# david3684/Prompt-Diffusion

Hardware: AMD Instinct MI355X
Metric: images/sec @ 512x512, 50-step DDIM, bs=8 (higher is better)
Workload: dtype f16; 1 GPU; SD1.5 UNet + Prompt-Diffusion ControlNet, 512x512, 50-step DDIM (eta 0), CFG 7.5, bs=8 per GPU (forward batch 16), random-init weights; global_batch=8, ddim_steps=50, parallelism=batch-shard x1, stream_f32=False, controlnet_stream_overlap=True

## Files before the change

### include/pdengine_ops.h

```cpp
#ifndef PDENGINE_OPS_H
#define PDENGINE_OPS_H
#include "pdengine.h"
#ifdef __cplusplus
extern "C" {
#endif
int pd_op_conv2d(pd_engine* e, const float* x, const float* w, const float* bias, const float* residual, int B, int Cin, int H,
                 int W, int Cout, int k, int stride, int upsample, int act_silu, float scale, int stream_out, float* y);
int pd_op_conv2d_upfold(pd_engine* e, const float* x, const float* w, const float* bias, const float* residual, int B, int Cin, int H,
                        int W, int Cout, float* y);
int pd_op_linear(pd_engine* e, const float* x, const float* w, const float* bias, int M, int K, int N, int geglu, int a_silu,
                 float* y);
typedef struct pd_gemm_ex_args {
    const float *x, *w, *bias, *residual, *rowvec, *gate, *ln_gamma, *ln_beta;
    int32_t M, K, N, act, a_silu, res_dt, out_dt, rows_per_sample;
    int32_t vt_begin, vt_extra, vt_tok_off, c_sample_rows, c_row_off, a_sample_rows, a_row_off, ldc_extra;
    float scale;
    float *y, *vt;
    int64_t touched;
} pd_gemm_ex_args;
int pd_op_linear_ex(pd_engine* e, pd_gemm_ex_args* a);
int pd_op_conv2d_ex(pd_engine* e, const float* x, const float* w, const float* bias, const float* residual, const float* rowvec, int B, int Cin,
                    int H, int W, int Cout, int k, int stride, int upsample, int act, float scale, int stream_out, float* y);
int pd_op_linear_fp8(pd_engine* e, const float* x, const float* w, const float* bias, int M, int K, int N, int act, float* y);
int pd_op_groupnorm(pd_engine* e, const float* x, const float* gamma, const float* beta, int B, int C, int H, int W, float eps,
                    int silu, float* y);
int pd_op_layernorm(pd_engine* e, const float* x, const float* gamma, const float* beta, int rows, int C, float* y);
int pd_op_groupnorm_slabs(pd_engine* e, const float* slabs, int nslab, const float* bias, const float* row, const float* gamma,
                          const float* beta, int B, int C, int H, int W, float eps, int silu, float* y);
int pd_op_groupnorm_coef(pd_engine* e, const float* x, const float* gamma, const float* beta, int B, int C, int H, int W, float eps,
                         float* coef);
int pd_op_ln_linear(pd_engine* e, int mode, const float* h, const float* x, const float* w1, const float* b1, const float* residual,
                    const float* gamma, const float* beta, const float* w, const float* bias, int M, int K, int N, float* h_out, float* y,
                    int* stats_parts, float* row_stats);
int pd_op_attention(pd_engine* e, const float* q, const float* k, const float* v, int B, int Nq, int Nk, int C, float* o);
int pd_op_attention_ex(pd_engine* e, const float* q, const float* k, const float* v, int B, int Nq, int Nk, int C, int heads, int causal,
                       float scale, const float* relbias, int layout, int vt_extra, float pad_fill, float* o, int64_t* touched);
int pd_op_vae_attention(pd_engine* e, const float* q, const float* k, const float* v, int B, int N, int C, float* o);
int pd_op_spatial_transformer(pd_engine* e, const char* prefix, const float* x, const float* context, int B, int H, int W, float* y);
int pd_op_spatial_transformer_ctx(pd_engine* e, const char* prefix, const float* x, const float* context, int B, int H, int W, int L, float* y);
int pd_op_time_embed(pd_engine* e, int net, const int64_t* t, int n, float* temb, float* emb);
int pd_op_timestep_embedding_i(const int64_t* t, int n, int dim, float* out);
int pd_op_timestep_embedding_f(const double* t, int n, int dim, float* out);
int pd_op_vae_downsample(pd_engine* e, const float* x, const float* w, const float* bias, int B, int C, int H, int W, float* y);
int pd_op_freeu_concat(pd_engine* e, const float* h, const float* h_add, const float* skip, const float* skip_add, int B, int C_h,
                       int C_skip, int H, int W, int skip_B, int skip_add_B, float s, float b, float* y);
int pd_op_hed_stage_tail(pd_engine* e, const float* x, const float* w, const float* bias, int B, int C, int H, int W, float* score,
                         float* pooled);
int pd_op_hed_fuse(pd_engine* e, const float* scores, const float* cw, const float* cb, int B, int H, int W, int what, float* out);
int pd_op_canny_hysteresis(pd_engine* e, const uint8_t* states, int B, int H, int W, int mem, uint8_t* out);
int pd_op_dwconv3x3(pd_engine* e, const float* x, const float* w, const float* bias, int B, int C, int H, int W, int stride, int in_relu6,
                    float* y);
int pd_op_upcat_bilinear(pd_engine* e, const float* x, int B, int C, int h, int w, int Cy, int c_off, float* y);
int pd_op_conv2d_dilated(pd_engine* e, const float* x, const float* w, const float* bias, int B, int Cin, int H, int W, int Cout, int dilation,
                         int relu, float* y);
int pd_op_mlsd_decode(pd_engine* e, const float* tp, int B, int h, int w, float thr_v, float thr_d, int32_t* segs, int32_t* count);
int pd_op_draw_lines(pd_engine* e, const int32_t* segs, const int32_t* count, int B, int n, int H, int W, uint8_t* out);
int pd_op_vae_tile_blend(pd_engine* e, const float* tiles, const pd_vae_tile* plan, int rows, int cols, int B, int C, int Cpad, int nchw,
                         float* out);
int pd_op_sd3_update(pd_engine* e, const float* v, const float* x, const float* z0, const float* mask, const float* eps, int B, int C,
                     int H, int W, int use_cfg, float guidance, float dsigma, float sigma, int pure, int seeded, int mem, float* x_out,
                     float* x_in_out);
#ifdef __cplusplus
}
#endif
#endif
```

### prompt-diffusion_amd/csrc/engine.cpp

```cpp
#include "engine.h"

#include <algorithm>
#include <climits>
#include <cmath>
#include <cstdarg>
#include <cstdio>
#include <cstring>

static thread_local char g_err[1024] = "";
void pd_set_error(const char* fmt, ...) {
    va_list ap;
    va_start(ap, fmt);
    vsnprintf(g_err, sizeof(g_err), fmt, ap);
    va_end(ap);
}
const char* pd_err_buf() { return g_err; }

static inline int round_up(int x, int m) { return (x + m - 1) / m * m; }

void* pd_engine::dmalloc(size_t bytes) {
    void* p = nullptr;
    if (bytes == 0) bytes = 16;
    if (hipMalloc(&p, bytes) != hipSuccess) { alloc_failed = true; return nullptr; }
    hipMemset(p, 0, bytes);
// ... 858 lines not shown

int pd_engine::gemm(const WMat& m, const Act& in, Act& out, const GemmCall& c) {
    PD_TRY(check_gemm(m, in, out, c));
    GemmParams p = fill_gemm(m, in, out, c);
    GemmPlan pl = plan_gemm(p, m, c);
    if (c.defer) c.defer->active = false;
    if (c.gn_coef && !pl.patch()) { pd_set_error("internal: fused GroupNorm requested for a conv that is not patch-eligible"); return 1; }
    const size_t mk = arena.mark();
    if (pl.splitk > 1) {
        p.slab = arena.alloc((size_t)pl.splitk * p.M * m.N * sizeof(float));
        if (!arena.dry && arena.top > arena.cap) {
            if (pl.patch()) { pd_set_error("no workspace for the conv split-K slabs"); return 1; }
            p.slab = nullptr; arena.overflow = false;
            pl = plan_gemm(p, m, c, false);
        }
    }
    p.splitk = pl.splitk; p.big_tile = pl.big_tile; p.defer_finalize = pl.defer_finalize ? 1 : 0;
    p.tile_cnt = pl.fused_tile_cnt ? tile_cnt : nullptr;
    if (pl.defer_finalize) c.defer->active = true;
    else arena.release(mk);
    if (pl.stats_parts) {
        LnStats& st = *c.ln_out;
        st.parts = p.stats_parts = pl.stats_parts; st.C = m.Nout; p.stats_out = st.stats;
        if (st.cap_parts && st.parts > st.cap_parts) { pd_set_error("internal: %d LayerNorm statistics partials per row, buffer holds %d", st.parts, st.cap_parts); return 1; }
    }
    if (arena.dry) return 0;
    PD_TRY(check_arena());
    const bool gemv = pl.family == GEMM_GEMV, ring = pl.family == GEMM_RING;
    ++launches;
    gemm_family = pl.family; gemm_splitk = p.splitk;
    gemm_ring_tile = ring ? pl.ring_tile : -1;
    gemm_tile = pl.family == GEMM_IGEMM ? gemm_launched_tile(p, in.dt == DT_FP8 ? PREC_FP8 : P) : 0;
    if (opt.gemm_tile >= 0 && pl.family == GEMM_IGEMM && gemm_tile != opt.gemm_tile) {
        pd_set_error("gemm: option gemm_tile %d, but this launch (mode, operands, epilogue, %d slices) has the tile %d instantiation only", opt.gemm_tile, p.splitk, gemm_tile);
        return 1;
    }
    ProfRec rec{};
    if (profiling && gemv) {
        prof_begin(rec, 1, 2.0 * (double)p.M * (double)m.Nout * (double)m.cin);
        rec.M = p.M; rec.N = p.N; rec.K = p.K; rec.taps = 10;
    } else if (profiling) {
        const double n_log = m.geglu ? 2.0 * m.Nout : (double)m.Nout;
        const bool upfold = pl.family == GEMM_UPFOLD;
        prof_begin(rec, pl.patch() || upfold ? 3 : m.taps == 9 ? 0 : 1, 2.0 * (double)p.M * n_log * (double)(upfold ? 4 : m.taps) * (double)m.cin);
        rec.M = p.M; rec.N = p.N; rec.K = upfold ? 4 * p.Cin : p.K; rec.taps = (upfold ? 4 : p.taps) * 10 + p.stride + (p.ups ? 5 : 0);
    }
    hipEvent_t mid = (profiling && !gemv && !pl.patch() && pl.family != GEMM_UPFOLD) ? next_event() : nullptr;
    if (gemv) {
        const int r = launch_gemv(reinterpret_cast<const float*>(in.p), in.C, m.w, T, m.Kpad, m.bias, reinterpret_cast<float*>(out.p), p.ldc,
                                  p.M, m.N, m.K, p.a_silu, stream);
        if (profiling) prof_end(rec);
        if (r) { pd_set_error("gemv launch failed"); return 1; }
        return 0;
    }
    static const char* const family_name[] = {"gemv", "patch1", "patch2", "patch4", "ring", "igemm", "upfold"};
    if (opt.verbose >= 2)
        fprintf(stderr, "[pdengine] gemm M %d N %d K %d taps %d stride %d ups %d: %s splitk %d big_tile %d ring_tile %d act %d R %d ln_in %d ln_out %d\n", p.M, p.N, p.K, p.taps,
                p.stride, p.ups, family_name[pl.family], p.splitk, p.big_tile, pl.ring_tile, p.act, p.R ? 1 : 0, p.ln_stats ? 1 : 0, p.stats_out ? 1 : 0);
    const int prec = in.dt == DT_FP8 ? PREC_FP8 : P;
    const int r = pl.family == GEMM_UPFOLD ? launch_conv_upfold(p, m.w_up, P, stream) : pl.family == GEMM_PATCH4 ? launch_conv_patch4(p, P, stream) : pl.family == GEMM_PATCH2 ? launch_conv_patch2(p, P, stream) :
                  pl.family == GEMM_PATCH1 ? launch_conv_patch(p, P, stream) : ring ? launch_ring_gemm(p, prec, pl.ring_tile, ncu, stream) : launch_gemm(p, prec, stream, mid);
    if (r) { pd_set_error("gemm launch failed: %s", hipGetErrorString(hipGetLastError())); return 1; }
    if (ring) ++ring_launches;
    if (pl.family == GEMM_UPFOLD) ++ups_fold_launches;
    if (pl.defer_finalize) *c.defer = SlabDefer{true, true, reinterpret_cast<const float*>(p.slab), p.splitk, p.bias, p.rowvec, p.rowvec_stride};
    if (profiling && mid && ring) HIP_OK(hipEventRecord(mid, stream));
    if (profiling) {
        if (mid) { rec.b = mid; prof.push_back(rec); }
        else prof_end(rec);
    }
    if (c.ln_out && !p.stats_out) {
        c.ln_out->parts = 1; c.ln_out->C = m.Nout;
        ++launches;
        if (launch_row_stats(out.p, out.dt, c.ln_out->stats, (int)out.rows(), out.C, stream)) { pd_set_error("row statistics launch failed"); return 1; }
    }
    return 0;
}

int pd_engine::conv(const ConvW& c, const Act& in, Act& out, GemmCall call) {
    call.stride = c.stride; call.pad_shift = c.pad_shift; call.dilation = c.dilation;
    return gemm(c.m, in, out, call);
}

int pd_engine::gn_stats(const Act& x, int& nchunk) {
    const int HW = x.H * x.W;
    nchunk = HW / 8;
    if (nchunk < 1) nchunk = 1;
    if (nchunk > 64) nchunk = 64;
    while ((size_t)x.B * nchunk * 32 * 2 * sizeof(double) > gn_partial_cap && nchunk > 1) nchunk /= 2;
    PD_LAUNCH(this, launch_gn_stats(x.p, x.dt, gn_partial, x.B, HW, x.C, 32, nchunk, stream), "groupnorm stats launch failed (C=%d)", x.C);
    return 0;
}

int pd_engine::groupnorm(const Act& x, Act& y, const float* g, const float* b, float eps, bool silu, const SlabDefer* from_slabs) {
    if (from_slabs && from_slabs->active) {
        if (!(opt.gn_single && gn_fused_bundle(x.dt, x.H * x.W, x.C, 32, opt.gn_reg))) { pd_set_error("internal: deferred split-K slabs without the single-kernel GroupNorm"); return 1; }
        if (arena.dry) return 0;
        PD_TRY(check_arena());
        ++launches;
        ++gn_from_slabs;
        if (launch_gn_fused_slabs(from_slabs->slabs, from_slabs->nslab, from_slabs->bias, from_slabs->rowvec, from_slabs->rowvec_stride, x.dt, y.p, y.dt, g, b,
                                  x.B, x.H * x.W, x.C, 32, eps, silu ? 1 : 0, opt.gn_reg, stream, &gn_kernel)) {
            pd_set_error("groupnorm (single kernel, split-K slabs) launch failed (C=%d)", x.C);
            return 1;
        }
        return 0;
    }
    if (opt.gn_single && gn_fused_bundle(x.dt, x.H * x.W, x.C, 32, opt.gn_reg)) {
        PD_LAUNCH(this, launch_gn_fused(x.p, x.dt, y.p, y.dt, g, b, x.B, x.H * x.W, x.C, 32, eps, silu ? 1 : 0, opt.gn_reg, stream, &gn_kernel),
                  "groupnorm (single kernel) launch failed (C=%d)", x.C);
        return 0;
    }
    int nchunk = 1;
    PD_TRY(gn_stats(x, nchunk));
    if (arena.dry) return 0;
    ++launches;
    gn_kernel = GN_KIND_TWO_PASS;
    if (launch_gn_apply(x.p, x.dt, y.p, y.dt, gn_partial, g, b, x.B, x.H * x.W, x.C, 32, nchunk, eps, silu ? 1 : 0, stream)) {
        pd_set_error("groupnorm launch failed (C=%d)", x.C);
        return 1;
    }
    return 0;
}

int pd_engine::conv_gn(const ConvW& c, const Act& x, Act& out, const float* g, const float* b, float eps, bool silu, GemmCall call,
                       const SlabDefer* in_slabs) {
    call.stride = c.stride; call.pad_shift = c.pad_shift; call.dilation = c.dilation;
    const bool fuse = opt.gn_fuse && x.C == c.m.cin_pad && patch_unsplit(patch_tiles(fill_gemm(c.m, x, out, call)));
    if (!fuse) {
        const size_t mk = arena.mark();
        Act a = new_act(x.B, x.H, x.W, x.C, T);
        PD_TRY(groupnorm(x, a, g, b, eps, silu, in_slabs));
        PD_TRY(gemm(c.m, a, out, call));
        if (!(call.defer && call.defer->active)) arena.release(mk);
        return 0;
    }
    if (in_slabs && in_slabs->active) { pd_set_error("internal: deferred split-K slabs in front of a GroupNorm-fused conv"); return 1; }
    int nchunk = 1;
    PD_TRY(gn_stats(x, nchunk));
    const size_t mk = arena.mark();
    float* coef = reinterpret_cast<float*>(arena.alloc((size_t)x.B * x.C * 2 * sizeof(float)));
    PD_LAUNCH(this, launch_gn_coef(gn_partial, g, b, coef, x.B, x.H * x.W, x.C, 32, nchunk, eps, stream), "groupnorm coefficient launch failed");
    call.gn_coef = coef; call.gn_silu = silu; call.defer = nullptr;
    PD_TRY(gemm(c.m, x, out, call));
    arena.release(mk);
    return 0;
}

int pd_engine::layernorm(const Act& x, Act& y, const float* g, const float* b, float eps) {
    PD_LAUNCH(this, launch_layernorm(x.p, x.dt, y.p, y.dt, g, b, (int)x.rows(), x.C, eps, stream), "layernorm launch failed (C=%d)", x.C);
    return 0;
}

int pd_engine::attention(const void* Q, int ldq, const void* K, int ldk, const void* VT, int vt_ld, void* O, int ldo, int B,
                         int Nq, int Nk, int C, int heads, bool causal, long long q_bs, long long k_bs, long long o_bs, const float* relbias,
                         float scale) {
    if (heads <= 0) heads = cfg.num_heads;
    if (arena.dry) return 0;
    PD_TRY(check_arena());
    AttnParams p{};
    p.Q = Q; p.K = K; p.VT = VT; p.O = O;
    p.ldq = ldq; p.ldk = ldk; p.ldo = ldo; p.vt_ld = vt_ld;
    p.q_bs = q_bs ? q_bs : (long long)Nq * ldq;
    p.k_bs = k_bs ? k_bs : (long long)Nk * ldk;
    p.vt_bs = (long long)C * vt_ld;
    p.o_bs = o_bs ? o_bs : (long long)Nq * ldo;
    p.Nq = Nq; p.Nk = Nk; p.heads = heads; p.dh = C / heads;
    p.causal = causal ? 1 : 0;
    p.scale = (float)(1.0 / std::sqrt((double)p.dh));
    if (scale != 0.f) p.scale = scale;
    p.B = B;
    p.legacy = opt.attn_legacy ? 1 : 0;
    ++launches;
    ProfRec rec{};
    if (profiling) {
        prof_begin(rec, 2, 4.0 * (double)B * heads * (double)Nq * (double)Nk * (double)p.dh);
        rec.M = Nq; rec.N = Nk; rec.K = p.dh; rec.taps = B;
    }
    const int r = relbias ? launch_attention_bias(p, relbias, P, stream, &attn_kernel) : launch_attention(p, P, stream, &attn_kernel);
    if (profiling) prof_end(rec);
    if (r) {
        pd_set_error(r == 2 ? "attention: unsupported head dim %d" : "attention launch failed (dh %d)", p.dh);
        return 1;
    }
    return 0;
}

int pd_engine::resblock(const ResW& r, const Act& x, Act& out, const float* embrow, int emb_stride) {
    out = new_act(x.B, x.H, x.W, r.cout, S);
    const size_t mk = arena.mark();
    Act h = new_act(x.B, x.H, x.W, r.cout, T);
    SlabDefer d;
    d.allow = opt.slab_gn && !opt.gn_fuse && opt.gn_single && h.dt == T && gn_fused_bundle(T, x.H * x.W, r.cout, 32, opt.gn_reg) > 0;
    PD_TRY(conv_gn(r.conv1, x, h, r.gn1_g, r.gn1_b, r.eps, true, {.rowvec = embrow, .rowvec_stride = emb_stride, .defer = &d}));
    Act skip = x;
    if (r.has_skip) {
        skip = new_act(x.B, x.H, x.W, r.cout, S);
        PD_TRY(conv(r.skip, x, skip));
    }
    PD_TRY(conv_gn(r.conv2, h, out, r.gn2_g, r.gn2_b, r.eps, true, {.R = &skip}, &d));
    arena.release(mk);
    return 0;
}

int pd_engine::transformer(const STW& s, const Act& x, Act& out, const KVSlot& kv, int out_B) {
    int B = x.B;
    const int H = x.H, W = x.W, C = s.C, N = H * W;
    if (out_B <= 0) out_B = B;
    if (out_B % B) { pd_set_error("internal: transformer output batch %d over %d shared samples", out_B, B); return 1; }
    const int reps = out_B / B;
    out = new_act(out_B, H, W, C, S);
    const size_t mk = arena.mark();
    const int L = kv.L > 0 ? kv.L : cfg.context_len, lpad = round_up(L, 8);
    const bool fused = st_tail_on(s, N, L) && s.tail_w && s.front_w && kv.P;
    const int npad = round_up(N, 8);
    Act h, qk, vt, ln;
    LnStats st0, st1;
    const bool fuse = (opt.ln_fuse < 0 ? !f32 : opt.ln_fuse != 0) && s.qkv.w_ln != nullptr;
    if (fused) {
        int nchunk = 1;
        PD_TRY(gn_stats(x, nchunk));
        float* coef = reinterpret_cast<float*>(arena.alloc((size_t)B * C * 2 * sizeof(float)));
        h = new_act(B, H, W, C, S);
        qk = new_act(B, H, W, 2 * C, T);
        vt = new_act(B, C, 1, npad, T);
        if (!arena.dry) {
            PD_TRY(check_arena());
            launches += 2;
            if (launch_gn_coef(gn_partial, s.gn_g, s.gn_b, coef, B, N, C, 32, nchunk, 1e-6f, stream)) {
                pd_set_error("groupnorm coefficient launch failed");
                return 1;
            }
            ProfRec rec{};
            if (profiling) {
                prof_begin(rec, 4, st_front_flops((long long)B * N));
                rec.M = B * N; rec.N = 4 * C; rec.K = C; rec.taps = 1;
            }
            const int r = launch_st_front(x.p, coef, h.p, qk.p, vt.p, s.front_w, s.front_vec, (long long)B * N, N, npad, P, stream);
            if (profiling) prof_end(rec);
            if (r) { pd_set_error("fused transformer-front launch failed: %s", hipGetErrorString(hipGetLastError())); return 1; }
        }
    } else {
    Act a = new_act(B, H, W, C, T);
    PD_TRY(groupnorm(x, a, s.gn_g, s.gn_b, 1e-6f, false));
    if (fuse) {
        st0.cap_parts = st1.cap_parts = ((C + 159) / 160) * 2;
        const size_t cap = (size_t)B * N * (size_t)st0.cap_parts * 2 * sizeof(float);
        st0.stats = reinterpret_cast<float*>(arena.alloc(cap));
        st1.stats = reinterpret_cast<float*>(arena.alloc(cap));
    }
    h = new_act(B, H, W, C, S);
    PD_TRY(gemm(s.proj_in.m, a, h, {.ln_out = fuse ? &st0 : nullptr}));
    if (!fuse) {
        ln = new_act(B, H, W, C, T);
        PD_TRY(layernorm(h, ln, s.ln_g[0], s.ln_b[0]));
    }
    qk = new_act(B, H, W, 2 * C, T);
    vt = new_act(B, C, 1, npad, T);
    PD_TRY(gemm(s.qkv, fuse ? h : ln, qk, {.VT = vt.p, .vt_begin = 2 * C, .vt_ld = npad, .ln_in = fuse ? &st0 : nullptr}));
    }
    Act att = new_act(B, H, W, C, T);
    const size_t eb = dt_size(T);
    PD_TRY(attention(qk.p, 2 * C, reinterpret_cast<char*>(qk.p) + (size_t)C * eb, 2 * C, vt.p, npad, att.p, C, B, N, N, C));
    if (fused) {
        if (!arena.dry) {
            PD_TRY(check_arena());
            ++launches;
            ProfRec rec{};
            if (profiling) {
                prof_begin(rec, 4, st_tail_flops((long long)out_B * N, L));
                rec.M = out_B * N; rec.N = C; rec.K = C; rec.taps = 0;
            }
            const int r = launch_st_tail(att.p, h.p, x.p, out.p, s.tail_w, s.tail_vec, kv.P, (long long)out_B * N, N, L, S,
                                         (float)(1.0 / std::sqrt((double)(C / cfg.num_heads))), P, stream, (long long)B * N);
            if (profiling) prof_end(rec);
            if (r) { pd_set_error("fused transformer-tail launch failed: %s", hipGetErrorString(hipGetLastError())); return 1; }
        }
// ... 71 lines not shown
    auto ctl = [&](int i) { return s0 ? batch_view(ses.control[i], s0, Bf) : ses.control[i]; };
    for (size_t i = 0; i < n.enc.size(); ++i) {
        EncBlock& b = n.enc[i];
        Act o;
        if (b.kind == 0) {
            o = new_act(x_in.B, x_in.H, x_in.W, b.cout, S);
            PD_TRY(conv(b.conv, x_in, o, {.R = &hint}));
        } else if (b.kind == 2) {
            o = new_act(h.B, h.H / 2, h.W / 2, b.cout, S);
            PD_TRY(conv(b.conv, h, o));
        } else {
            PD_TRY(resblock(b.res, h, o, emb_ptr(ses.emb_c, b.res, emb_row), emb_stride ? b.res.cout : 0));
            if (b.attn) {
                Act o2;
                PD_TRY(transformer(b.st, o, o2, kvs(b.st), Bf));
                o = o2;
            }
        }
        h = o;
        Act c = ctl((int)i);
        if (c.B != h.B) { pd_set_error("internal: control tensor %d sized for batch %d, block output has %d", (int)i, c.B, h.B); return 1; }
        PD_TRY(conv(n.zero[i], h, c, {.scale = scales ? scales[i] : 1.f}));
    }
    Act m0, m1, m2;
    PD_TRY(resblock(n.mid0, h, m0, emb_ptr(ses.emb_c, n.mid0, emb_row), emb_stride ? n.mid0.cout : 0));
    PD_TRY(transformer(n.mid1, m0, m1, kvs(n.mid1), Bf));
    PD_TRY(resblock(n.mid2, m1, m2, emb_ptr(ses.emb_c, n.mid2, emb_row), emb_stride ? n.mid2.cout : 0));
    const int last = (int)n.enc.size();
    Act cl = ctl(last);
    PD_TRY(conv(n.mid_out, m2, cl, {.scale = scales ? scales[last] : 1.f}));
    return 0;
}

Act pd_engine::batch_view(const Act& a, int first, int count) {
    Act v = a;
    v.p = reinterpret_cast<char*>(a.p) + (size_t)first * a.H * a.W * a.C * dt_size(a.dt);
    v.B = count;
    return v;
}

int pd_engine::run_unet(const Act& x_in_full, int emb_row, int emb_stride, bool only_mid, Act& eps) {
    NetW& n = unet;
    std::vector<Act> hs;
    Act h;
    const int Bf = x_in_full.B;
    Act x_in = x_in_full;
    if (ses.share_u) x_in.B = Bf / 2;
    for (size_t i = 0; i < n.enc.size(); ++i) {
        EncBlock& b = n.enc[i];
        Act o;
        if (b.kind == 0) {
            o = new_act(x_in.B, x_in.H, x_in.W, b.cout, S);
            PD_TRY(conv(b.conv, x_in, o));
        } else if (b.kind == 2) {
            o = new_act(h.B, h.H / 2, h.W / 2, b.cout, S);
            PD_TRY(conv(b.conv, h, o));
        } else {
            PD_TRY(resblock(b.res, h, o, emb_ptr(ses.emb_u, b.res, emb_row), emb_stride ? b.res.cout : 0));
            if (b.attn) {
                Act o2;
                PD_TRY(transformer(b.st, o, o2, ses.kv_u[b.st.kv_slot], Bf));
                o = o2;
            }
        }
        h = o;
        hs.push_back(h);
    }
    Act m0, m1, m2;
    PD_TRY(resblock(n.mid0, h, m0, emb_ptr(ses.emb_u, n.mid0, emb_row), emb_stride ? n.mid0.cout : 0));
    PD_TRY(transformer(n.mid1, m0, m1, ses.kv_u[n.mid1.kv_slot], Bf));
    PD_TRY(resblock(n.mid2, m1, m2, emb_ptr(ses.emb_u, n.mid2, emb_row), emb_stride ? n.mid2.cout : 0));
    h = m2;
    PD_TRY(join_controlnet());
    const int nctl = (int)cnet.enc.size();
    for (size_t i = 0; i < n.dec.size(); ++i) {
        DecBlock& b = n.dec[i];
        Act skip = hs.back();
        hs.pop_back();
        Act cat = new_act(h.B, h.H, h.W, h.C + skip.C, S);
        const Act* a_add = i == 0 ? &ses.control[nctl] : nullptr;
        const Act* b_add = only_mid ? nullptr : &ses.control[nctl - 1 - (int)i];
        const int stage = (int)i / (cfg.num_res_blocks + 1);
        const bool fu = stage < 2 && freeu_on();
        PD_LAUNCH(this,
                  fu ? launch_freeu_concat(h.p, a_add ? a_add->p : nullptr, skip.p, b_add ? b_add->p : nullptr, cat.p, S, h.B, h.H, h.W, h.C, skip.C,
                                           freeu[stage], freeu[2 + stage], stream, skip.rows(), b_add ? b_add->rows() : 0)
                     : launch_concat_add(h.p, a_add ? a_add->p : nullptr, skip.p, b_add ? b_add->p : nullptr, cat.p, S, h.rows(), h.C, skip.C, stream,
                                         skip.rows(), b_add ? b_add->rows() : 0),
                  fu ? "FreeU concat launch failed" : "concat launch failed");
        Act o;
        PD_TRY(resblock(b.res, cat, o, emb_ptr(ses.emb_u, b.res, emb_row), emb_stride ? b.res.cout : 0));
        if (b.attn) {
            Act o2;
            PD_TRY(transformer(b.st, o, o2, ses.kv_u[b.st.kv_slot]));
            o = o2;
        }
        if (b.up) {
            Act o3 = new_act(o.B, o.H * 2, o.W * 2, o.C, S);
            PD_TRY(conv(b.upconv, o, o3, {.ups = 1}));
            o = o3;
        }
        h = o;
    }
    eps = new_act(h.B, h.H, h.W, round_up(cfg.out_channels, 4), DT_F32);
    PD_TRY(conv_gn(n.outconv, h, eps, n.out_g, n.out_b, 1e-5f, true));
    return 0;
}

void pd_engine::swap_context() {
    std::swap(arena, arena2);
    std::swap(stream, stream2);
    std::swap(gn_partial, gn_partial2);
    std::swap(tile_cnt, tile_cnt2);
}

int pd_engine::join_controlnet() {
    const pd_sample_args& a = ses.a;
    if (arena.dry) return 0;
    if (cn_pending) {
        HIP_OK(hipStreamWaitEvent(stream, ev_join, 0));
        cn_pending = false;
    }
    if (a.guess_mode && a.use_cfg) {
        for (size_t i = 0; i <= cnet.enc.size(); ++i)
            HIP_OK(hipMemsetAsync(ses.control[i].p, 0, ses.control[i].bytes() / 2, stream));
    }
    return 0;
}

int pd_engine::forward_eps(int emb_row, int emb_stride, const float* scales, Act& eps) {
    const pd_sample_args& a = ses.a;
    const int Bf = ses.Bf;
    Act x_in;
    x_in.p = ses.x_in; x_in.B = Bf; x_in.H = a.h; x_in.W = a.w; x_in.C = 8; x_in.dt = DT_F32;
    const bool share = opt.cfg_share && a.use_cfg && emb_stride == 0 && Bf % 2 == 0;
    ses.share_u = share;
    ses.share_c = share && ses.hint_shared && !a.guess_mode;
    ses.cn_cond_only = opt.cfg_share && a.guess_mode && a.use_cfg && emb_stride == 0 && Bf % 2 == 0;
    int hh = a.h, ww = a.w;
    bool front = ses.share_c;
    for (size_t i = 0; i < cnet.enc.size(); ++i) {
        if (cnet.enc[i].kind == 2) { hh /= 2; ww /= 2; }
        if (cnet.enc[i].attn) front = false;
        ses.control[i] = new_act(front ? Bf / 2 : Bf, hh, ww, cnet.enc[i].cout, S);
    }
    ses.control[cnet.enc.size()] = new_act(Bf, hh, ww, cnet.enc.back().cout, S);
    const bool two = opt.two_streams && stream2 != nullptr;
    if (two && !arena.dry) {
        HIP_OK(hipEventRecord(ev_fork, stream));
        HIP_OK(hipStreamWaitEvent(stream2, ev_fork, 0));
    }
    if (two) swap_context();
    const size_t mk = arena.mark();
    int rc = run_controlnet(x_in, emb_row, emb_stride, scales);
    arena.release(mk);
    if (two) {
        if (!rc && !arena.dry && hipEventRecord(ev_join, stream) != hipSuccess) rc = 1;
        swap_context();
    }
    if (rc) return rc;
    cn_pending = two;
    PD_TRY(run_unet(x_in, emb_row, emb_stride, a.only_mid_control != 0, eps));
    return 0;
}
```

### prompt-diffusion_amd/csrc/engine.h

```cpp
#pragma once
#include <cstdint>
#include <map>
#include <string>
#include <unordered_map>
#include <vector>

#include "../../include/pdengine.h"
#include "options.h"
#include "pd_common.h"

void pd_set_error(const char* fmt, ...);
void pd_host_timestep_embedding(const int64_t* t, int n, int dim, std::vector<float>& out);
void pd_host_timestep_embedding_f(const double* t, int n, int dim, std::vector<float>& out);
int pd_lms_table(const pd_config& cfg, const pd_lms_args& u, const int64_t* ts, int n, std::vector<double>& rows, std::vector<double>& times);
int pd_resample_axis(int in_size, int out_size, int filter, int* ksize, std::vector<int32_t>& bounds, std::vector<int32_t>& kk);
int pd_unipc_table(const pd_config& cfg, const pd_unipc_args& u, const int64_t* ts, int n, std::vector<double>& coef);

#define HIP_OK(expr)                                                                            \
    do {                                                                                        \
        hipError_t _e = (expr);                                                                 \
        if (_e != hipSuccess) {                                                                 \
            pd_set_error("%s failed: %s (%s:%d)", #expr, hipGetErrorString(_e), __FILE__, __LINE__); \
            return 1;                                                                           \
        }                                                                                       \
// ... 381 lines not shown
    float* x_state = nullptr;
    float* x_in = nullptr;
    float* pred_x0 = nullptr;
    float* eps_g = nullptr;
    float* noise = nullptr;
    bool noise_seeded = false;
    void* ctx = nullptr;
    Act hint;
    std::vector<KVSlot> kv_u, kv_c;
    std::vector<float*> emb_u, emb_c;
    int emb_rows = 0;
    float* per_step = nullptr;
    Act control[PD_NUM_CONTROL];
    size_t session_top = 0;
    bool hint_shared = false, share_u = false, share_c = false;
    bool cn_cond_only = false;
    int solver = 0;
    std::vector<double> unipc_coef;
    int unipc_ring = 0;
    double* u_last = nullptr;
    double* u_ring[3] = {nullptr, nullptr, nullptr};
    std::vector<double> lms_coef;
    std::vector<double> lms_times;
    std::vector<int> lms_step;
    std::vector<int> lms_pushed;
    int lms_ring = 0;
    bool lms_keep = false;
    double* l_keep = nullptr;
    double* l_ring[3] = {nullptr, nullptr, nullptr};
    int rows() const { return solver == SOLVER_LMS ? (int)lms_times.size() : S; }
    float* init_z0 = nullptr;
    float* init_eps = nullptr;
    float* mask = nullptr;
    std::vector<BlendCoef> blend;
};

struct pd_engine {
    pd_config cfg{};
    int device = 0;
    int ncu = 256;
    hipStream_t stream = nullptr;
    void* comm = nullptr;
    int comm_world = 1, comm_rank = 0;
    bool f32 = false;
    int P = DT_BF16;
    int T = DT_BF16;
    int S = DT_BF16;
    std::vector<Param> params;
    std::unordered_map<std::string, int> index;
    NetW unet, cnet;
    VaeW vae;
    VaeEncW vae_enc;
    ClipW text;
    struct GraphEntry { uint64_t key; hipGraph_t graph; hipGraphExec_t exec; };
    std::vector<GraphEntry> graphs;
    void clear_graphs();
    int run_steps_graph();
    WeightGroup reg_group = GROUP_SAMPLER;
    int missing(WeightGroup g) const;
    int require_loaded(WeightGroup g, const char* what);
    std::vector<void*> owned;
    bool alloc_failed = false;
    int check_arena();
    size_t weight_bytes = 0;
    Arena arena;
    Arena arena2;
    hipStream_t stream2 = nullptr;
    double* gn_partial2 = nullptr;
    int* tile_cnt2 = nullptr;
    hipEvent_t ev_fork = nullptr, ev_join = nullptr;
    bool cn_pending = false;
    EngineOptions opt;
    float freeu[4] = {0.f, 0.f, 0.f, 0.f};
    bool freeu_on() const { return freeu[0] != 0.f && freeu[1] != 0.f && freeu[2] != 0.f && freeu[3] != 0.f; }
    uint32_t* rng_dev = nullptr;
    uint32_t rng_host[4] = {0u, 0u, 0u, 0u};
    uint64_t rng_seed = 0, rng_base = 0;
    long long graph_captures = 0, graph_replays = 0;
    void swap_context();
    int join_controlnet();
    Session ses;
    long long launches = 0;
    long long gn_from_slabs = 0;
    long long ring_launches = 0;
    int gn_kernel = 0;
    long long ups_fold_launches = 0;
    int attn_kernel = 0;
    int gemm_tile = -1, gemm_splitk = -1;
    int gemm_ring_tile = -1;
    int gemm_family = -1;
    struct ProfRec { hipEvent_t a, b; int klass; double flops; int M, N, K, taps; };
    bool profiling = false;
    float prof_overhead_ms = 0.f;
    std::vector<ProfRec> prof;
    std::vector<hipEvent_t> ev_pool;
    size_t ev_used = 0;
    hipEvent_t next_event();
    void prof_begin(ProfRec& r, int klass, double flops);
    void prof_end(ProfRec& r);
    double* gn_partial = nullptr;
    int* tile_cnt = nullptr;
    static constexpr int kTileCnt = 4096;
    size_t gn_partial_cap = 0;

    int build();
    void* dmalloc(size_t bytes);
    void make_mat(WMat& m, int n_rows, int k_logical, int taps, int cin, bool bias, bool geglu = false);
    void reg_mat(const std::string& name, std::vector<int64_t> shape, WMat* m, int row_off, bool conv);
    void reg_vec(const std::string& name, int n, float** dst, char init);
    void reg_bias(const std::string& name, WMat* m, int off, int n, bool geglu = false);
    void build_conv(const std::string& prefix, ConvW& c, int cin, int cout, int k, int stride);
    void build_res(const std::string& prefix, ResW& r, int cin, int cout, NetW& net);
    void build_st(const std::string& prefix, STW& s, int ch, NetW& net);
    void build_encoder(const std::string& prefix, NetW& net);
    void build_middle(const std::string& prefix, NetW& net);
    void build_vres(const std::string& prefix, ResW& r, int cin, int cout, bool diffusers = false);
    void build_vattn(const std::string& prefix, VaeAttnW& a, int C, bool diffusers = false);
    void build_vae();
    void build_vae_encoder();
    void build_vae_decoder(VaeW& v, const std::string& prefix);
    void build_vae_encoder(VaeEncW& v, const std::string& prefix);
    VaeW sd3_vae;
    VaeEncW sd3_vae_enc;
    long long vae_flash_launches = 0;
    bool vae_flash_on(const VaeDesc& d, int C, long long N) const;
    int vae_forward(VaeW& v, const float* latents_dev, int B, int h, int w, float* out_dev, float scale, float shift);
    int vae_encoder_forward(VaeEncW& v, const float* images_dev, int B, int H, int W, int what, const float* noise_dev, float* out_dev, float scale,
                            float shift);
    int vae_attention(const VaeAttnW& a, const VaeDesc& d, const Act& x, Act& out);
    int vae_attn_product(const void* qk, int ld, const void* vt, int npad, void* att, int B, int N, int C, bool flash, float* sc, void* pr);
    int vae_decode_layers(VaeW& v, const Act& z, Act& img);
    int vae_encode_layers(VaeEncW& v, const Act& x, Act& mom);
    int vae_decode_call(VaeW& v, int which, const float* latents, int B, int h, int w, int mem, float scale, float shift, float* images_out);
    int vae_encode_call(VaeEncW& v, int which, const float* images, int B, int H, int W, int mem, int what, const float* noise, float scale,
                        float shift, float* out);
    struct VaeTiling { bool tiling = false, slicing = false; int tile = 0; double overlap = 0.0; int batch = 0; };
    VaeTiling vae_tiling[2];
    bool vae_tile_odd_flash = false;
    std::vector<char> vae_tile_blob;
    long long vae_tiles_run = 0;
    VaeTilePlan vae_plan_for(int which, int h, int w, int u, bool encode) const;
    int vae_check_tiles(const VaeTilePlan& p, const VaeDesc& d, int C, const char* who) const;
    int vae_tile_setup(const VaeTilePlan& p, int B, int cpad, VaeTileRun& run);
    int vae_tile_blend(const VaeTilePlan& p, const VaeTileRun& run, int B, int C, int cpad, bool nchw, float* out);
    int vae_decode_managed(VaeW& v, int which, const float* src, int B, int h, int w, float* dout, float scale, float shift);
    int vae_encode_managed(VaeEncW& v, int which, const float* src, int B, int H, int W, int what, const float* noise, float* dout, float scale,
                           float shift);
    template <class Body> int side_call(const char* what, Body&& body);
    int side_grow(const char* what, size_t need);
    template <class Check, class Build> int configure(const char* who, WeightGroup g, Check&& check, Build&& build);
    template <class Build> int configure(const char* who, WeightGroup g, Build&& build) { return configure(who, g, [] { return 0; }, build); }

    void build_clip(const std::string& prefix, ClipW& w);
    void build_clip_layers(const std::string& prefix, ClipW& w);
    void build_text();
    int clip_embed(const ClipW& w, const int* ids_dev, Act& x);
    int self_attention(const WMat& qkv, const Act& ln, int inner, int heads, bool causal, const float* relbias, float scale, Act& att);
    int clip_block(const TextLayerW& l, Act& x, int heads, Activation act, bool causal, float eps = 1e-5f);
    int clip_blocks(const ClipW& w, int first, int last, Act& x);
    int text_forward(const int* ids_dev, int B, float* out_dev, int clip_skip);

    HedW hed;
    void build_hed();
    int hed_forward(const float* images_dev, int B, int H, int W, int what, float* out_dev);

    MlsdW mlsd;
// ... 35 lines not shown

    pd_sd3_config sd3{};
    Sd3NetW sd3_tr, sd3_cn;
    std::vector<hipEvent_t> sd3_ev;
    struct Sd3Io {
        const float *latents, *context, *pooled, *cond, *pair;
        const float* cn_pooled;
        const float* t_host;
        int B, H, W, S;
        float scale;
    };
    void build_sd3_net(const std::string& prefix, Sd3NetW& net, bool controlnet);
    int sd3_embed(Sd3NetW& net, const Sd3Io& io, bool controlnet, Act& hs, Act& c, Act& modbuf);
    int sd3_block(const Sd3BlockW& b, Act& x, Act& c, const Act& modbuf, const Act& qk, const Act& vt, const Act* pre_add = nullptr);
    int sd3_forward(const Sd3Io& io, float* v_out_dev, int control_index, float* control_out_dev);
    ClipW sd3_clip[2];
    Sd3T5W sd3_t5;
    int sd3_text_joint = 0;
    std::vector<int32_t> t5_bucket_host;
    void build_sd3_t5(const std::string& prefix);
    int sd3_clip_forward(ClipW& w, const int* ids_dev, int B, int clip_skip, float* hid, int hid_rows, int hid_ld, int c_off, int width,
                         float* pooled, int pooled_ld);
    int sd3_t5_forward(const int* ids_dev, int B, int Lt, float* out, int out_rows, int row_off);
    int t5_block(const T5LayerW& l, Act& x, const float* relbias);
    int rmsnorm(const Act& x, void* y, int y_dt, const float* w, float eps, int y_sample_rows = 0, int y_row_off = 0, int y_ld = 0);
    bool sd3_fp8_dirty = true;
    int sd3_quantize();

    struct LoraEntry { int adapter = 0, r = 0; };
    struct LoraForm {
        int adapter = 0, kind = 0, r1 = 0, r2 = 0, ka = 0, kb = 0;
        float* buf = nullptr;
        size_t bytes = 0;
        float *ut1 = nullptr, *d1 = nullptr, *ut2 = nullptr, *d2 = nullptr, *mag = nullptr;
    };
    struct LoraTarget {
        void* w0 = nullptr;
        size_t w0_bytes = 0;
        float* ut = nullptr;
        float* d = nullptr;
        int R = 0;
        std::vector<LoraEntry> entries;
        std::vector<float> merged;
        std::vector<LoraForm> forms;
        std::vector<float> fmerged;
    };
    float* lora_tmp = nullptr;
    float* lora_sum = nullptr;
    size_t lora_tmp_cap = 0;
    int lora_add_ex(int adapter, const char* name, const pd_lora_factors& f);
    int lora_target_base(int pi);
    std::map<int, LoraTarget> lora;
    std::map<int, float> lora_scale;
    float* lora_scale_dev = nullptr;
    size_t lora_scale_cap = 0;
    int lora_add(int adapter, const char* name, const float* up, int up_rows, int rank, const float* down, const int64_t* down_shape,
                 int down_ndim);
    int lora_set_scales(const float* scales, int n);
    int lora_remove(int adapter);
    int lora_merge(int only_param, bool force);
    int lora_rebase(int only_param);
    void lora_release();
    size_t lora_bytes(bool base_only) const;
    int read_param(const Param& p, float* out);

    int load(const char* name, const void* data, const int64_t* shape, int ndim, int dtype);
    int init_random(uint64_t seed);
    int upload_vec(float* dst_dev, const float* src, int n, bool geglu, int half);
    int upload_rows(WMat& m, int row_off, const float* src, int rows, bool conv);

    Act new_act(int B, int H, int W, int C, int dt);
    int gemm(const WMat& m, const Act& in, Act& out, const GemmCall& c = {});
    int check_gemm(const WMat& m, const Act& in, const Act& out, const GemmCall& c) const;
    static GemmParams fill_gemm(const WMat& m, const Act& in, const Act& out, const GemmCall& c);
    GemmPlan plan_gemm(const GemmParams& p, const WMat& m, const GemmCall& c, bool allow_splitk = true) const;
    ChipFill chip_fill() const { return ChipFill(opt, ncu); }
    int patch_tiles(const GemmParams& p) const; bool patch_unsplit(int ptiles) const;
    int fold_upconv(WMat& m);
    int fold_upconvs();
    bool upfold_wanted(const WMat& m) const;
    int fold_layernorms();
    bool ln_dirty = true;
    bool st_tail_on(const STW& s, int rows_per_sample, int L) const;
    int gn_stats(const Act& x, int& nchunk);
    int conv(const ConvW& c, const Act& in, Act& out, GemmCall call = {});
    int conv_gn(const ConvW& c, const Act& x, Act& out, const float* g, const float* b, float eps, bool silu, GemmCall call = {},
                const SlabDefer* in_slabs = nullptr);
    int groupnorm(const Act& x, Act& y, const float* g, const float* b, float eps, bool silu, const SlabDefer* from_slabs = nullptr);
    int layernorm(const Act& x, Act& y, const float* g, const float* b, float eps = 1e-5f);
    int resblock(const ResW& r, const Act& x, Act& out, const float* embrow, int emb_stride);
    int transformer(const STW& s, const Act& x, Act& out, const KVSlot& kv, int out_B = 0);
    int repeat_act(const Act& src, int reps, Act& dst);
    static Act batch_view(const Act& a, int first, int count);
    int attention(const void* Q, int ldq, const void* K, int ldk, const void* VT, int vt_ld, void* O, int ldo, int B, int Nq,
                  int Nk, int C, int heads = 0, bool causal = false, long long q_bs = 0, long long k_bs = 0, long long o_bs = 0,
                  const float* relbias = nullptr, float scale = 0.f);

    int run_controlnet(const Act& x_in, int emb_row, int emb_stride, const float* scales);
    int run_unet(const Act& x_in, int emb_row, int emb_stride, bool only_mid, Act& eps);
    int forward_eps(int emb_row, int emb_stride, const float* scales, Act& eps);

    int ensure_arena(int rows, bool per_step);
    int session_setup(const pd_sample_args& a, const int64_t* t_rows, int n_rows, bool want_per_step, const double* t_rows_f = nullptr);
    int compute_emb(NetW& net, std::vector<float*>& tabs, const int64_t* t, int n, int row0, const double* tf = nullptr);
    int begin(const pd_sample_args* a, bool want_per_step, const pd_unipc_args* u = nullptr, const pd_lms_args* l = nullptr);
    int step(int i);
    UpdateState update_state(const Act& eps) const;
    int step_ddim(int i, const UpdateState& u, const BlendArgs* bl);
    int step_unipc(int i, const UpdateState& u, const BlendArgs* bl);
    int step_lms(int i, const UpdateState& u, const BlendArgs* bl);
    int make_schedule(int steps, float eta, std::vector<int64_t>& ts, std::vector<float>& a, std::vector<float>& ap,
                      std::vector<float>& sg, std::vector<float>& s1m, const int64_t* custom_desc = nullptr);
};

struct Bracket {
    pd_engine* e;
    pd_engine::ProfRec rec{};
    const bool on;
    Bracket(pd_engine* e_, int klass) : e(e_), on(klass >= 0 && e_->profiling && !e_->arena.dry) {
        if (on) e->prof_begin(rec, klass, 0.0);
    }
    ~Bracket() {
        if (on) e->prof_end(rec);
    }
};

struct RegGroup {
    pd_engine& e;
    RegGroup(pd_engine& e_, int g) : e(e_) { e.reg_group = (WeightGroup)g; }
    ~RegGroup() { e.reg_group = GROUP_SAMPLER; }
};

struct SideCall {
    pd_engine& e;
    template <class T> T* scratch(size_t n) { return reinterpret_cast<T*>(e.arena.alloc(n * sizeof(T))); }
    template <class T> int src(const T** dev, const T* p, size_t n, int mem) {
        *dev = p;
        if (mem == PD_MEM_DEVICE) return 0;
        T* d = scratch<T>(n);
        *dev = d;
        return upload(d, p, n * sizeof(T));
    }
    int upload(void* dev, const void* host, size_t bytes);
    template <class T> T* dst(T* p, size_t n, int mem, size_t rows = 1, size_t pitch = 0) {
        return reinterpret_cast<T*>(stage(p, n * sizeof(T), rows, pitch * sizeof(T), mem));
    }
    void* stage(void* p, size_t width, size_t rows, size_t pitch, int mem);
    int finish();
    struct Back { void* dst; const void* src; size_t width, rows, pitch; int mem; };
    std::vector<Back> backs;
};

template <class Body>
int pd_engine::side_call(const char* what, Body&& body) {
    SideCall f{*this};
    std::swap(arena, arena2);
    const Arena saved = arena;
    arena.base = nullptr; arena.cap = 0; arena.top = 0; arena.peak = 0; arena.dry = true;
    int r = body(f);
    const size_t need = arena.peak + (64u << 20);
    arena = saved;
    arena.dry = false;
    if (!r) r = side_grow(what, need);
    if (!r) {
        arena.top = 0; arena.peak = 0;
        r = body(f);
        if (!r) r = f.finish();
        else hipStreamSynchronize(stream);
        arena.top = 0;
    }
    std::swap(arena, arena2);
    return r;
}
// ... 15 lines not shown
```

### prompt-diffusion_amd/csrc/norm.hip

```cpp
#include <type_traits>

#include "pd_common.h"


namespace {

constexpr int GN_THREADS = 256;

__device__ __forceinline__ void gn_run_flush(double& ds, double& dq, float s, float q, float pq, float pivot, int n) {
    const float sd = s - (float)n * pivot;
    const float dev = pq - sd * sd / (float)n;
    const bool refine = n >= 8 && q > 8.f * dev;
    const double p = (double)pivot, np = (double)n * p, d = (double)s - np;
    ds += (double)s;
    dq += refine ? (double)pq + p * (2.0 * d + np) : (double)q;
}

template <int XD>
__global__ __launch_bounds__(GN_THREADS) void gn_stats_kernel(const void* __restrict__ x, double* __restrict__ partial,
                                                               int HW, int C, int groups, int nchunk) {
    constexpr bool XF32 = XD == DT_F32;
    constexpr int VEC = XF32 ? 4 : 8;
    __shared__ double s_sum[64], s_sq[64];
    const int b = blockIdx.y, chunk = blockIdx.x;
    const int tid = threadIdx.x;
    if (tid < 64) { s_sum[tid] = 0.0; s_sq[tid] = 0.0; }
    __syncthreads();
    const int ppc = (HW + nchunk - 1) / nchunk;
    const int p0 = chunk * ppc, p1 = min(HW, p0 + ppc);
    const int nvec = C / VEC;
    const int lanes = min(nvec, GN_THREADS);
    const int rows_par = GN_THREADS / lanes;
    const int pr = tid / lanes, vc = tid - pr * lanes;
    const int cpg = C / groups;
    if (pr < rows_par) {
        for (int v = vc; v < nvec; v += lanes) {
            float s[VEC], q[VEC];
#pragma unroll
            for (int j = 0; j < VEC; ++j) { s[j] = 0.f; q[j] = 0.f; }
            double ds[VEC], dq[VEC];
#pragma unroll
            for (int j = 0; j < VEC; ++j) { ds[j] = 0.0; dq[j] = 0.0; }
            [[maybe_unused]] float pv[VEC], pq[VEC];
            int cnt = 0;
            for (int p = p0 + pr; p < p1; p += rows_par) {
                const size_t idx = ((size_t)b * HW + p) * C + (size_t)v * VEC;
                float f[VEC];
                if constexpr (XF32) {
                    const f32x4 t = *reinterpret_cast<const f32x4*>(reinterpret_cast<const float*>(x) + idx);
#pragma unroll
                    for (int j = 0; j < 4; ++j) f[j] = t[j];
                } else {
                    const uint4 t = *reinterpret_cast<const uint4*>(reinterpret_cast<const uint16_t*>(x) + idx);
                    unpack8<XD>(t, f);
                }
                if constexpr (XF32) {
#pragma unroll
                    for (int j = 0; j < VEC; ++j) { const double d = (double)f[j]; ds[j] += d; dq[j] = fma(d, d, dq[j]); }
                } else {
                    if constexpr (XD == DT_F16) {
                        if (cnt == 0) {
#pragma unroll
                            for (int j = 0; j < VEC; ++j) { pv[j] = f[j]; pq[j] = 0.f; }
                        }
#pragma unroll
                        for (int j = 0; j < VEC; ++j) { const float d = f[j] - pv[j]; pq[j] = fmaf(d, d, pq[j]); }
                    }
#pragma unroll
                    for (int j = 0; j < VEC; ++j) { s[j] += f[j]; q[j] = fmaf(f[j], f[j], q[j]); }
                    if (++cnt == 16) {
#pragma unroll
                        for (int j = 0; j < VEC; ++j) {
                            if constexpr (XD == DT_F16) gn_run_flush(ds[j], dq[j], s[j], q[j], pq[j], pv[j], 16);
                            else { ds[j] += s[j]; dq[j] += q[j]; }
                            s[j] = 0.f; q[j] = 0.f;
                        }
                        cnt = 0;
                    }
                }
            }
#pragma unroll
            for (int j = 0; j < VEC; ++j) {
                if constexpr (XD == DT_F16) {
                    if (cnt) gn_run_flush(ds[j], dq[j], s[j], q[j], pq[j], pv[j], cnt);
                } else {
                    ds[j] += s[j];
                    dq[j] += q[j];
                }
                const int g = (v * VEC + j) / cpg;
                atomicAdd(&s_sum[g], ds[j]);
                atomicAdd(&s_sq[g], dq[j]);
            }
        }
    }
    __syncthreads();
    if (tid < groups) {
        double* o = partial + (((size_t)b * nchunk + chunk) * groups + tid) * 2;
        o[0] = s_sum[tid];
        o[1] = s_sq[tid];
    }
}

template <int XD, int YD>
__global__ __launch_bounds__(GN_THREADS) void gn_apply_kernel(const void* __restrict__ x, void* __restrict__ y,
                                                               const double* __restrict__ partial,
                                                               const float* __restrict__ gamma, const float* __restrict__ beta,
                                                               int HW, int C, int groups, int nchunk, int napply,
                                                               float eps, int do_silu) {
    constexpr bool XF32 = XD == DT_F32, YF32 = YD == DT_F32;
    constexpr int VEC = XF32 ? 4 : 8;
    __shared__ float s_mean[64], s_rstd[64];
    __shared__ double s_part[4][64][2];
    const int b = blockIdx.y;
    const int tid = threadIdx.x;
    {
        const int g = tid & 63, part = tid >> 6;
        if (g < groups) {
            double s = 0.0, q = 0.0;
            for (int c = part; c < nchunk; c += 4) {
                const double* o = partial + (((size_t)b * nchunk + c) * groups + g) * 2;
                s += o[0];
                q += o[1];
            }
            s_part[part][g][0] = s;
            s_part[part][g][1] = q;
        }
    }
    __syncthreads();
    if (tid < groups) {
        const double s = (s_part[0][tid][0] + s_part[1][tid][0]) + (s_part[2][tid][0] + s_part[3][tid][0]);
        const double q = (s_part[0][tid][1] + s_part[1][tid][1]) + (s_part[2][tid][1] + s_part[3][tid][1]);
        const double n = (double)HW * (double)(C / groups);
        const double mean = s / n;
        double var = q / n - mean * mean;
        var = var < 0.0 ? 0.0 : var;
        s_mean[tid] = (float)mean;
        s_rstd[tid] = (float)(1.0 / sqrt(var + (double)eps));
    }
    __syncthreads();
    const int cpg = C / groups;
    const int nvec = C / VEC;
    const int lanes = min(nvec, GN_THREADS);
    const int rows_par = GN_THREADS / lanes;
    const int pr = tid / lanes, vc = tid - pr * lanes;
    if (pr >= rows_par) return;
    const int ppc = (HW + napply - 1) / napply;
    const int p0 = blockIdx.x * ppc, p1 = min(HW, p0 + ppc);
    const char* xb = reinterpret_cast<const char*>(x) + (size_t)b * HW * C * (XF32 ? 4 : 2);
    char* yb = reinterpret_cast<char*>(y) + (size_t)b * HW * C * (YF32 ? 4 : 2);
    for (int v = vc; v < nvec; v += lanes) {
        float ka[VEC], kb[VEC];
#pragma unroll
        for (int j = 0; j < VEC; ++j) {
            const int c = v * VEC + j;
            const int g = c / cpg;
            ka[j] = s_rstd[g] * gamma[c];
            kb[j] = beta[c] - s_mean[g] * ka[j];
        }
        for (int p = p0 + pr; p < p1; p += rows_par) {
            const size_t e = (size_t)p * C + (size_t)v * VEC;
            const uint4 raw = *reinterpret_cast<const uint4*>(xb + e * (XF32 ? 4 : 2));
            float f[VEC];
            if constexpr (XF32) {
                const float* t = reinterpret_cast<const float*>(&raw);
#pragma unroll
                for (int j = 0; j < 4; ++j) f[j] = t[j];
            } else {
                unpack8<XD>(raw, f);
            }
#pragma unroll
            for (int j = 0; j < VEC; ++j) {
                float r = fmaf(f[j], ka[j], kb[j]);
                f[j] = do_silu ? silu_f(r) : r;
            }
            if constexpr (YF32) {
                float* o = reinterpret_cast<float*>(yb) + e;
#pragma unroll
                for (int h = 0; h < VEC / 4; ++h) *reinterpret_cast<f32x4*>(o + 4 * h) = f32x4{f[4 * h], f[4 * h + 1], f[4 * h + 2], f[4 * h + 3]};
            } else {
                uint16_t* o = reinterpret_cast<uint16_t*>(yb) + e;
                if constexpr (VEC == 8) {
                    *reinterpret_cast<uint4*>(o) = pack8<YD>(f);
                } else {
                    uint2 u;
                    u.x = pack2<YD>(f[0], f[1]); u.y = pack2<YD>(f[2], f[3]);
                    *reinterpret_cast<uint2*>(o) = u;
                }
            }
        }
    }
}

constexpr int GNF_THREADS = 960;

struct GnSlabSrc { const float* slabs; long long slab_stride; const float* bias; const float* row; int nslab, row_stride; };

template <int XD, int YD, bool SLAB = false>
__global__ __launch_bounds__(GNF_THREADS) void gn_fused_kernel(const void* __restrict__ x, void* __restrict__ y,
                                                                const float* __restrict__ gamma, const float* __restrict__ beta,
                                                                int HW, int C, int groups, int BC, float eps, int do_silu, GnSlabSrc src) {
    constexpr bool XF32 = XD == DT_F32, YF32 = YD == DT_F32;
    constexpr int VEC = XF32 ? 4 : 8;
    constexpr int EX = XF32 ? 4 : 2;
    extern __shared__ __attribute__((aligned(16))) char slab[];
    const int nb = C / BC;
    const int bid = xcd_tile_order(blockIdx.x, gridDim.x);
    const int b = bid / nb, bundle = bid - b * nb;
    const int tid = threadIdx.x;
    const int nvec = BC / VEC;
    const int v = tid % nvec, pr = tid / nvec;
    const int rows_par = GNF_THREADS / nvec;
    const int cpg = C / groups, gpb = BC / cpg;
    const int c0 = bundle * BC + v * VEC;
    double* red = reinterpret_cast<double*>(slab + (size_t)HW * BC * EX);
    const char* xb = reinterpret_cast<const char*>(x) + ((size_t)b * HW * C + c0) * EX;

    double ds[VEC], dq[VEC];
    float s[VEC], q[VEC];
#pragma unroll
    for (int j = 0; j < VEC; ++j) { ds[j] = 0.0; dq[j] = 0.0; s[j] = 0.f; q[j] = 0.f; }
    [[maybe_unused]] float pv[VEC], pq[VEC];
    int cnt = 0;
    for (int p = pr; p < HW; p += rows_par) {
        uint4 raw;
        if constexpr (SLAB) {
            const float* sp = src.slabs + ((size_t)b * HW + p) * C + c0;
            float acc[VEC];
#pragma unroll
            for (int j = 0; j < VEC; j += 4) {
                f32x4 t = *reinterpret_cast<const f32x4*>(sp + j);
                for (int k = 1; k < src.nslab; ++k) t += *reinterpret_cast<const f32x4*>(sp + (size_t)k * src.slab_stride + j);
                if (src.bias) t += *reinterpret_cast<const f32x4*>(src.bias + c0 + j);
                if (src.row) t += *reinterpret_cast<const f32x4*>(src.row + (size_t)b * src.row_stride + c0 + j);
                acc[j] = t[0]; acc[j + 1] = t[1]; acc[j + 2] = t[2]; acc[j + 3] = t[3];
            }
            if constexpr (XF32) raw = make_uint4(__float_as_uint(acc[0]), __float_as_uint(acc[1]), __float_as_uint(acc[2]), __float_as_uint(acc[3]));
            else raw = pack8<XD>(acc);
        } else {
            raw = *reinterpret_cast<const uint4*>(xb + (size_t)p * C * EX);
        }
        *reinterpret_cast<uint4*>(slab + ((size_t)p * nvec + v) * 16) = raw;
        float f[VEC];
        if constexpr (XF32) {
            const float* t = reinterpret_cast<const float*>(&raw);
#pragma unroll
            for (int j = 0; j < 4; ++j) f[j] = t[j];
        } else {
            unpack8<XD>(raw, f);
        }
        if constexpr (XF32) {
#pragma unroll
            for (int j = 0; j < VEC; ++j) { const double d = (double)f[j]; ds[j] += d; dq[j] = fma(d, d, dq[j]); }
        } else {
            if constexpr (XD == DT_F16) {
                if (cnt == 0) {
#pragma unroll
                    for (int j = 0; j < VEC; ++j) { pv[j] = f[j]; pq[j] = 0.f; }
                }
#pragma unroll
                for (int j = 0; j < VEC; ++j) { const float d = f[j] - pv[j]; pq[j] = fmaf(d, d, pq[j]); }
            }
#pragma unroll
            for (int j = 0; j < VEC; ++j) { s[j] += f[j]; q[j] = fmaf(f[j], f[j], q[j]); }
            if (++cnt == 16) {
#pragma unroll
                for (int j = 0; j < VEC; ++j) {
                    if constexpr (XD == DT_F16) gn_run_flush(ds[j], dq[j], s[j], q[j], pq[j], pv[j], 16);
                    else { ds[j] += s[j]; dq[j] += q[j]; }
                    s[j] = 0.f; q[j] = 0.f;
                }
                cnt = 0;
            }
        }
    }
    if constexpr (XD == DT_F16) {
        if (cnt) {
#pragma unroll
            for (int j = 0; j < VEC; ++j) { gn_run_flush(ds[j], dq[j], s[j], q[j], pq[j], pv[j], cnt); s[j] = 0.f; q[j] = 0.f; }
        }
    }
    double gs[4] = {0.0, 0.0, 0.0, 0.0}, gq[4] = {0.0, 0.0, 0.0, 0.0};
#pragma unroll
    for (int j = 0; j < VEC; ++j) {
        const int g = (v * VEC + j) / cpg;
        const double a = ds[j] + s[j], bq = dq[j] + q[j];
#pragma unroll
        for (int k = 0; k < 4; ++k) if (k == g) { gs[k] += a; gq[k] += bq; }
    }
#pragma unroll
    for (int k = 0; k < 4; ++k)
#pragma unroll
        for (int o = 32; o > 0; o >>= 1) { gs[k] += __shfl_xor(gs[k], o); gq[k] += __shfl_xor(gq[k], o); }
    if ((tid & 63) == 0) {
#pragma unroll
        for (int k = 0; k < 4; ++k) { red[((tid >> 6) * 4 + k) * 2] = gs[k]; red[((tid >> 6) * 4 + k) * 2 + 1] = gq[k]; }
    }
    __syncthreads();
    __shared__ float s_mean[4], s_rstd[4];
    if (tid < gpb) {
        double S = 0.0, Q = 0.0;
        for (int t = 0; t < GNF_THREADS / 64; ++t) { S += red[(t * 4 + tid) * 2]; Q += red[(t * 4 + tid) * 2 + 1]; }
        const double n = (double)HW * (double)cpg;
        const double mean = S / n;
        double var = Q / n - mean * mean;
        var = var < 0.0 ? 0.0 : var;
        s_mean[tid] = (float)mean;
        s_rstd[tid] = (float)(1.0 / sqrt(var + (double)eps));
    }
// ... 98 lines not shown
        }
    }
#pragma unroll
    for (int o = 32; o > 0; o >>= 1) s += __shfl_xor(s, o);
    const float mean = s / (float)C;
    float q = 0.f;
#pragma unroll
    for (int k = 0; k < MAXV; ++k) {
        const int vi = lane + 64 * k;
        if (vi < nvec4) {
#pragma unroll
            for (int j = 0; j < 4; ++j) { const float d = v[k][j] - mean; q = fmaf(d, d, q); }
        }
    }
#pragma unroll
    for (int o = 32; o > 0; o >>= 1) q += __shfl_xor(q, o);
    const float rstd = 1.0f / sqrtf(q / (float)C + eps);
#pragma unroll
    for (int k = 0; k < MAXV; ++k) {
        const int vi = lane + 64 * k;
        if (vi < nvec4) {
            const f32x4 g = *reinterpret_cast<const f32x4*>(gamma + vi * 4);
            const f32x4 be = *reinterpret_cast<const f32x4*>(beta + vi * 4);
            f32x4 o;
#pragma unroll
            for (int j = 0; j < 4; ++j) o[j] = (v[k][j] - mean) * rstd * g[j] + be[j];
            store4(y, (size_t)row * C + (size_t)vi * 4, YD, o);
        }
    }
}

template <int XD>
__global__ __launch_bounds__(256) void row_stats_kernel(const void* __restrict__ x, float* __restrict__ stats, int rows, int C) {
    const int lane = threadIdx.x & 63;
    const int row = blockIdx.x * 4 + (threadIdx.x >> 6);
    if (row >= rows) return;
    float s = 0.f, q = 0.f;
    for (int v = lane; v < C / 4; v += 64) {
        const f32x4 t = load4(x, (size_t)row * C + (size_t)v * 4, XD);
        s += (t[0] + t[1]) + (t[2] + t[3]);
        q += (t[0] * t[0] + t[1] * t[1]) + (t[2] * t[2] + t[3] * t[3]);
    }
#pragma unroll
    for (int o = 32; o > 0; o >>= 1) { s += __shfl_xor(s, o); q += __shfl_xor(q, o); }
    if (lane == 0) { stats[(size_t)row * 2] = s; stats[(size_t)row * 2 + 1] = q; }
}

template <int DT>
__global__ __launch_bounds__(256) void ln_fold_kernel(const void* __restrict__ W, void* __restrict__ Wout, int N, int K, int Kpad,
                                                      const float* __restrict__ gamma, const float* __restrict__ beta,
                                                      const float* __restrict__ bias_in, float* __restrict__ colsum,
                                                      float* __restrict__ bias_out) {
    const int lane = threadIdx.x & 63;
    const int n = blockIdx.x * 4 + (threadIdx.x >> 6);
    if (n >= N) return;
    float cs = 0.f, bs = 0.f;
    for (int k = lane; k < Kpad; k += 64) {
        float w, wg = 0.f;
        const size_t i = (size_t)n * Kpad + k;
        if constexpr (DT == DT_F32) w = reinterpret_cast<const float*>(W)[i];
        else w = cvt32<DT>(reinterpret_cast<const uint16_t*>(W)[i]);
        if (k < K) {
            wg = w * gamma[k];
            bs += beta[k] * w;
        }
        if constexpr (DT == DT_F32) {
            reinterpret_cast<float*>(Wout)[i] = wg;
        } else {
            const uint16_t r = cvt16<DT>(wg);
            reinterpret_cast<uint16_t*>(Wout)[i] = r;
            wg = cvt32<DT>(r);
        }
        cs += wg;
    }
#pragma unroll
    for (int o = 32; o > 0; o >>= 1) { cs += __shfl_xor(cs, o); bs += __shfl_xor(bs, o); }
    if (lane == 0) {
        colsum[n] = cs;
        bias_out[n] = (bias_in ? bias_in[n] : 0.f) + bs;
    }
}


template <int XD, int VB, int NL, bool SLAB>
__global__ __launch_bounds__(NL == 16 ? 512 : 1024) void gn_reg_kernel(const void* __restrict__ x, void* __restrict__ y, const float* __restrict__ gamma,
                                                       const float* __restrict__ beta, int HW, int C, int groups, int nv, float eps,
                                                       int do_silu, GnSlabSrc src) {
    constexpr int EV = VB / 2;
    constexpr int NW = VB / 4;
    __shared__ double red[16][2];
    const int bid = xcd_tile_order(blockIdx.x, gridDim.x);
    const int b = bid / groups, g = bid - b * groups;
    const int tid = threadIdx.x;
    const int v = tid % nv, pr = tid / nv;
    const int cpg = C / groups;
    const int c0 = g * cpg + v * EV;
    unsigned raw[NL][NW];
    const char* xb = reinterpret_cast<const char*>(x) + ((size_t)b * HW * C + c0) * 2;
#pragma unroll
    for (int i = 0; i < NL; ++i) {
        const int p = pr + 64 * i;
        if constexpr (SLAB) {
            static_assert(!SLAB || EV >= 4, "slab input comes in 4-channel pieces");
            const float* sp = src.slabs + ((size_t)b * HW + p) * C + c0;
            float acc[EV];
#pragma unroll
            for (int j = 0; j < EV; j += 4) {
                f32x4 t = *reinterpret_cast<const f32x4*>(sp + j);
                for (int k = 1; k < src.nslab; ++k) t += *reinterpret_cast<const f32x4*>(sp + (size_t)k * src.slab_stride + j);
                if (src.bias) t += *reinterpret_cast<const f32x4*>(src.bias + c0 + j);
                if (src.row) t += *reinterpret_cast<const f32x4*>(src.row + (size_t)b * src.row_stride + c0 + j);
                acc[j] = t[0]; acc[j + 1] = t[1]; acc[j + 2] = t[2]; acc[j + 3] = t[3];
            }
#pragma unroll
            for (int w = 0; w < NW; ++w) raw[i][w] = pack2<XD>(acc[2 * w], acc[2 * w + 1]);
        } else {
            const char* q = xb + (size_t)p * C * 2;
            if constexpr (NW == 4) {
                const uint4 t = *reinterpret_cast<const uint4*>(q);
                raw[i][0] = t.x; raw[i][1] = t.y; raw[i][2] = t.z; raw[i][3] = t.w;
            } else if constexpr (NW == 2) {
                const uint2 t = *reinterpret_cast<const uint2*>(q);
                raw[i][0] = t.x; raw[i][1] = t.y;
            } else {
                raw[i][0] = *reinterpret_cast<const unsigned*>(q);
            }
        }
    }
    float s[EV], q2[EV];
#pragma unroll
    for (int j = 0; j < EV; ++j) { s[j] = 0.f; q2[j] = 0.f; }
    constexpr bool PIV = XD == DT_F16 && NL >= 8;
    [[maybe_unused]] float pv[EV], pq[EV];
    if constexpr (PIV) {
#pragma unroll
        for (int w = 0; w < NW; ++w) unpack2<XD>(raw[0][w], pv[2 * w], pv[2 * w + 1]);
#pragma unroll
        for (int j = 0; j < EV; ++j) pq[j] = 0.f;
    }
#pragma unroll
    for (int i = 0; i < NL; ++i)
#pragma unroll
        for (int w = 0; w < NW; ++w) {
            float lo, hi;
            unpack2<XD>(raw[i][w], lo, hi);
            s[2 * w] += lo; q2[2 * w] = fmaf(lo, lo, q2[2 * w]);
            s[2 * w + 1] += hi; q2[2 * w + 1] = fmaf(hi, hi, q2[2 * w + 1]);
            if constexpr (PIV) {
                lo -= pv[2 * w]; hi -= pv[2 * w + 1];
                pq[2 * w] = fmaf(lo, lo, pq[2 * w]);
                pq[2 * w + 1] = fmaf(hi, hi, pq[2 * w + 1]);
            }
        }
    double gs = 0.0, gq = 0.0;
#pragma unroll
    for (int j = 0; j < EV; ++j) {
        if constexpr (PIV) gn_run_flush(gs, gq, s[j], q2[j], pq[j], pv[j], NL);
        else { gs += (double)s[j]; gq += (double)q2[j]; }
    }
#pragma unroll
    for (int o = 32; o > 0; o >>= 1) { gs += __shfl_xor(gs, o); gq += __shfl_xor(gq, o); }
    if ((tid & 63) == 0) { red[tid >> 6][0] = gs; red[tid >> 6][1] = gq; }
    __syncthreads();
    double S = 0.0, Q = 0.0;
    for (int t = 0; t < nv; ++t) { S += red[t][0]; Q += red[t][1]; }
    const double n = (double)HW * (double)cpg;
    const double mean = S / n;
    double var = Q / n - mean * mean;
    var = var < 0.0 ? 0.0 : var;
    const float mean_f = (float)mean, rstd_f = (float)(1.0 / sqrt(var + (double)eps));
    float ka[EV], kb[EV];
#pragma unroll
    for (int j = 0; j < EV; ++j) {
        ka[j] = rstd_f * gamma[c0 + j];
        kb[j] = beta[c0 + j] - mean_f * ka[j];
    }
    char* yb = reinterpret_cast<char*>(y) + ((size_t)b * HW * C + c0) * 2;
#pragma unroll
    for (int i = 0; i < NL; ++i) {
        unsigned out[NW];
#pragma unroll
        for (int w = 0; w < NW; ++w) {
            float lo, hi;
            unpack2<XD>(raw[i][w], lo, hi);
            float r0 = fmaf(lo, ka[2 * w], kb[2 * w]), r1 = fmaf(hi, ka[2 * w + 1], kb[2 * w + 1]);
            if (do_silu) { r0 = silu_f(r0); r1 = silu_f(r1); }
            out[w] = pack2<XD>(r0, r1);
        }
        char* o = yb + (size_t)(pr + 64 * i) * C * 2;
        if constexpr (NW == 4) *reinterpret_cast<uint4*>(o) = make_uint4(out[0], out[1], out[2], out[3]);
        else if constexpr (NW == 2) *reinterpret_cast<uint2*>(o) = make_uint2(out[0], out[1]);
        else *reinterpret_cast<unsigned*>(o) = out[0];
    }
}

static int gn_reg_vb(int x_dt, int y_dt, int HW, int C, int groups, bool slab) {
    if (x_dt != y_dt || (x_dt != DT_F16 && x_dt != DT_BF16) || C % groups) return 0;
    if (HW != 64 && HW != 256 && HW != 1024) return 0;
    const int gb = (C / groups) * 2;
    const int nv_max = HW == 1024 ? 8 : 16;
    for (int vb = 16; vb >= (slab ? 8 : 4); vb >>= 1)
        if (gb % vb == 0 && gb / vb <= nv_max && (C * 2) % vb == 0) return vb;
    return 0;
}

template <bool SLAB>
static int launch_gn_reg(const void* x, int dt, void* y, const float* gamma, const float* beta, int B, int HW, int C, int groups, float eps,
                         int do_silu, const GnSlabSrc& src, hipStream_t s) {
    const int vb = gn_reg_vb(dt, dt, HW, C, groups, true);
    if (!vb) return 1;
    const int nv = (C / groups) * 2 / vb, nl = HW / 64;
    const dim3 grid(B * groups), block(64 * nv);
    bool done = false;
    auto go = [&](auto XD, auto VB, auto NL) {
        if constexpr (SLAB && decltype(VB)::value < 8) return;
        else {
            hipLaunchKernelGGL((gn_reg_kernel<decltype(XD)::value, decltype(VB)::value, decltype(NL)::value, SLAB>), grid, block, 0, s, x, y, gamma, beta,
                               HW, C, groups, nv, eps, do_silu, src);
            done = true;
        }
    };
    auto by_nl = [&](auto XD, auto VB) {
        if (nl == 1) go(XD, VB, std::integral_constant<int, 1>{});
        else if (nl == 4) go(XD, VB, std::integral_constant<int, 4>{});
        else go(XD, VB, std::integral_constant<int, 16>{});
    };
    auto by_vb = [&](auto XD) {
        if (vb == 16) by_nl(XD, std::integral_constant<int, 16>{});
        else if (vb == 8) by_nl(XD, std::integral_constant<int, 8>{});
        else by_nl(XD, std::integral_constant<int, 4>{});
    };
    if (dt == DT_F16) by_vb(std::integral_constant<int, DT_F16>{});
    else by_vb(std::integral_constant<int, DT_BF16>{});
    return done && hipGetLastError() == hipSuccess ? 0 : 1;
}

template <typename F>
bool dispatch_xy(int x_dt, int y_dt, F&& f) {
    using IF = std::integral_constant<int, DT_F32>;
    using IB = std::integral_constant<int, DT_BF16>;
    using IH = std::integral_constant<int, DT_F16>;
    if (x_dt == DT_F32 && y_dt == DT_F32) f(IF{}, IF{});
    else if (x_dt == DT_F32 && y_dt == DT_BF16) f(IF{}, IB{});
    else if (x_dt == DT_F32 && y_dt == DT_F16) f(IF{}, IH{});
    else if (x_dt == DT_BF16 && y_dt == DT_F32) f(IB{}, IF{});
    else if (x_dt == DT_F16 && y_dt == DT_F32) f(IH{}, IF{});
    else if (x_dt == DT_BF16 && y_dt == DT_BF16) f(IB{}, IB{});
    else if (x_dt == DT_F16 && y_dt == DT_F16) f(IH{}, IH{});
    else return false;
    return true;
}

}

int launch_gn_stats(const void* x, int x_dt, double* partial, int B, int HW, int C, int groups, int nchunk, hipStream_t s) {
    if (groups > 64 || C % groups || C % 8) return 1;
    dim3 grid(nchunk, B);
    if (x_dt == DT_F32)
        hipLaunchKernelGGL(gn_stats_kernel<DT_F32>, grid, dim3(GN_THREADS), 0, s, x, partial, HW, C, groups, nchunk);
    else if (x_dt == DT_F16)
        hipLaunchKernelGGL(gn_stats_kernel<DT_F16>, grid, dim3(GN_THREADS), 0, s, x, partial, HW, C, groups, nchunk);
    else
        hipLaunchKernelGGL(gn_stats_kernel<DT_BF16>, grid, dim3(GN_THREADS), 0, s, x, partial, HW, C, groups, nchunk);
    return hipGetLastError() == hipSuccess ? 0 : 1;
}

int launch_gn_apply(const void* x, int x_dt, void* y, int y_dt, const double* partial, const float* gamma,
                    const float* beta, int B, int HW, int C, int groups, int nchunk, float eps, int silu, hipStream_t s) {
    int napply = (1024 + B - 1) / B;
    if (napply > HW / 16) napply = HW / 16;
    if (napply < 1) napply = 1;
    dim3 grid(napply, B);
    const bool ok = dispatch_xy(x_dt, y_dt, [&](auto XD, auto YD) {
        hipLaunchKernelGGL((gn_apply_kernel<decltype(XD)::value, decltype(YD)::value>), grid, dim3(GN_THREADS), 0, s, x, y, partial,
                           gamma, beta, HW, C, groups, nchunk, napply, eps, silu);
    });
    return ok && hipGetLastError() == hipSuccess ? 0 : 1;
}

static int gn_slab_bundle(int x_dt, int HW, int C, int groups);
int gn_fused_bundle(int x_dt, int HW, int C, int groups, bool reg) {
    if (C % groups) return 0;
    if (reg && gn_reg_vb(x_dt, x_dt, HW, C, groups, true)) return C / groups;
    return gn_slab_bundle(x_dt, HW, C, groups);
}
static int gn_slab_bundle(int x_dt, int HW, int C, int groups) {
    const int VEC = x_dt == DT_F32 ? 4 : 8, EX = x_dt == DT_F32 ? 4 : 2;
    if (C % groups) return 0;
    const int cpg = C / groups;
    int BC = cpg;
    while (BC % VEC) BC += cpg;
    if (C % BC || BC / cpg > 4 || GNF_THREADS % (BC / VEC)) return 0;
    const size_t bytes = (size_t)HW * BC * EX + (GNF_THREADS / 64) * 4 * 2 * sizeof(double);
    return bytes <= 100 * 1024 ? BC : 0;
}

int launch_gn_fused(const void* x, int x_dt, void* y, int y_dt, const float* gamma, const float* beta, int B, int HW, int C, int groups,
                    float eps, int do_silu, bool reg, hipStream_t s, int* kind) {
    if (kind) *kind = 0;
    if (reg && gn_reg_vb(x_dt, y_dt, HW, C, groups, true)) {
        if (kind) *kind = GN_KIND_REGISTER;
        return launch_gn_reg<false>(x, x_dt, y, gamma, beta, B, HW, C, groups, eps, do_silu, GnSlabSrc{}, s);
    }
    const int BC = gn_slab_bundle(x_dt, HW, C, groups);
    if (!BC) return 1;
    if (kind) *kind = GN_KIND_LDS_SLAB;
    const int EX = x_dt == DT_F32 ? 4 : 2;
    const size_t smem = (size_t)HW * BC * EX + (GNF_THREADS / 64) * 4 * 2 * sizeof(double);
    const dim3 grid(B * (C / BC));
    bool fail = false;
    const bool ok = dispatch_xy(x_dt, y_dt, [&](auto XD, auto YD) {
        static unsigned long long attr_done = 0;
        auto kfn = gn_fused_kernel<decltype(XD)::value, decltype(YD)::value>;
        if (ensure_dyn_smem(reinterpret_cast<const void*>(kfn), 104 * 1024, &attr_done)) { fail = true; return; }
        hipLaunchKernelGGL(kfn, grid, dim3(GNF_THREADS), smem, s, x, y, gamma, beta, HW, C, groups, BC, eps, do_silu, GnSlabSrc{});
    });
    return ok && !fail && hipGetLastError() == hipSuccess ? 0 : 1;
}

int launch_gn_fused_slabs(const float* slabs, int nslab, const float* bias, const float* rowvec, int rowvec_stride, int x_dt, void* y, int y_dt,
                          const float* gamma, const float* beta, int B, int HW, int C, int groups, float eps, int do_silu, bool reg, hipStream_t s, int* kind) {
    if (kind) *kind = 0;
    if (!slabs || nslab < 1 || C % 4) return 1;
    if (reg && gn_reg_vb(x_dt, y_dt, HW, C, groups, true)) {
        if (kind) *kind = GN_KIND_REGISTER;
        return launch_gn_reg<true>(nullptr, x_dt, y, gamma, beta, B, HW, C, groups, eps, do_silu,
                                   GnSlabSrc{slabs, (long long)B * HW * C, bias, rowvec, nslab, rowvec_stride}, s);
    }
    const int BC = gn_slab_bundle(x_dt, HW, C, groups);
    if (!BC) return 1;
    if (kind) *kind = GN_KIND_LDS_SLAB;
    const int EX = x_dt == DT_F32 ? 4 : 2;
    const size_t smem = (size_t)HW * BC * EX + (GNF_THREADS / 64) * 4 * 2 * sizeof(double);
    const dim3 grid(B * (C / BC));
    const GnSlabSrc src{slabs, (long long)B * HW * C, bias, rowvec, nslab, rowvec_stride};
    bool fail = false;
    const bool ok = dispatch_xy(x_dt, y_dt, [&](auto XD, auto YD) {
        static unsigned long long attr_done = 0;
        auto kfn = gn_fused_kernel<decltype(XD)::value, decltype(YD)::value, true>;
        if (ensure_dyn_smem(reinterpret_cast<const void*>(kfn), 104 * 1024, &attr_done)) { fail = true; return; }
        hipLaunchKernelGGL(kfn, grid, dim3(GNF_THREADS), smem, s, static_cast<const void*>(nullptr), y, gamma, beta, HW, C, groups, BC, eps, do_silu, src);
    });
    return ok && !fail && hipGetLastError() == hipSuccess ? 0 : 1;
}

int launch_gn_coef(const double* partial, const float* gamma, const float* beta, float* coef, int B, int HW, int C, int groups,
                   int nchunk, float eps, hipStream_t s) {
    hipLaunchKernelGGL(gn_coef_kernel, dim3(B), dim3(256), 0, s, partial, gamma, beta, coef, HW, C, groups, nchunk, eps);
    return hipGetLastError() == hipSuccess ? 0 : 1;
}

int launch_row_stats(const void* x, int x_dt, float* stats, int rows, int C, hipStream_t s) {
    if (C % 4) return 1;
    dim3 grid((rows + 3) / 4);
    if (x_dt == DT_F32) hipLaunchKernelGGL(row_stats_kernel<DT_F32>, grid, dim3(256), 0, s, x, stats, rows, C);
    else if (x_dt == DT_F16) hipLaunchKernelGGL(row_stats_kernel<DT_F16>, grid, dim3(256), 0, s, x, stats, rows, C);
    else hipLaunchKernelGGL(row_stats_kernel<DT_BF16>, grid, dim3(256), 0, s, x, stats, rows, C);
    return hipGetLastError() == hipSuccess ? 0 : 1;
}

int launch_ln_fold(const void* W, void* Wout, int dt, int N, int K, int Kpad, const float* gamma, const float* beta, const float* bias_in,
                   float* colsum, float* bias_out, hipStream_t s) {
    dim3 grid((N + 3) / 4);
    if (dt == DT_F32) hipLaunchKernelGGL(ln_fold_kernel<DT_F32>, grid, dim3(256), 0, s, W, Wout, N, K, Kpad, gamma, beta, bias_in, colsum, bias_out);
    else if (dt == DT_F16) hipLaunchKernelGGL(ln_fold_kernel<DT_F16>, grid, dim3(256), 0, s, W, Wout, N, K, Kpad, gamma, beta, bias_in, colsum, bias_out);
    else hipLaunchKernelGGL(ln_fold_kernel<DT_BF16>, grid, dim3(256), 0, s, W, Wout, N, K, Kpad, gamma, beta, bias_in, colsum, bias_out);
    return hipGetLastError() == hipSuccess ? 0 : 1;
}

int launch_layernorm(const void* x, int x_dt, void* y, int y_dt, const float* gamma, const float* beta, int rows,
                     int C, float eps, hipStream_t s) {
    if (C % 4 || C > 64 * 4 * 8) return 1;
    dim3 grid((rows + 3) / 4);
    const int nv = (C / 4 + 63) / 64;
    const bool ok = dispatch_xy(x_dt, y_dt, [&](auto XD, auto YD) {
        constexpr int xd = decltype(XD)::value, yd = decltype(YD)::value;
        if (nv <= 2) hipLaunchKernelGGL((layernorm_kernel<xd, yd, 2>), grid, dim3(256), 0, s, x, y, gamma, beta, rows, C, eps);
        else if (nv <= 5) hipLaunchKernelGGL((layernorm_kernel<xd, yd, 5>), grid, dim3(256), 0, s, x, y, gamma, beta, rows, C, eps);
        else hipLaunchKernelGGL((layernorm_kernel<xd, yd, 8>), grid, dim3(256), 0, s, x, y, gamma, beta, rows, C, eps);
    });
    return ok && hipGetLastError() == hipSuccess ? 0 : 1;
}
```

### prompt-diffusion_amd/csrc/ops_abi.cpp

```cpp
#include <cmath>
#include <cstring>
#include <string>
#include <vector>

#include "../../include/pdengine_ops.h"
#include "engine.h"

namespace {
struct DevBuf {
    void* p = nullptr;
    explicit DevBuf(size_t bytes) { if (hipMalloc(&p, bytes ? bytes : 16) != hipSuccess) p = nullptr; else { hipMemset(p, 0, bytes ? bytes : 16); hipDeviceSynchronize(); } }
    ~DevBuf() { if (p) hipFree(p); }
};
struct TempMat {
    pd_engine* e;
    size_t owned0;
    explicit TempMat(pd_engine* e_) : e(e_), owned0(e_->owned.size()) {}
    ~TempMat() {
        while (e->owned.size() > owned0) { hipFree(e->owned.back()); e->owned.pop_back(); }
    }
};
int to_dev_nhwc(pd_engine* e, const float* host, void* dst, int dt, int B, int C, int H, int W, int Cpad) {
    DevBuf tmp((size_t)B * C * H * W * 4);
    if (!tmp.p) return 1;
// ... 57 lines not shown
    if (!e || !x || !w || !y) { pd_set_error("null argument"); return 1; }
    if (B < 1 || Cin < 1 || Cout < 1 || H < 1 || W < 1) { pd_set_error("pd_op_conv2d_upfold: need B, Cin, Cout, H, W >= 1"); return 1; }
    HIP_OK(hipSetDevice(e->device));
    TempMat guard(e);
    ConvW c;
    c.cin = Cin; c.cout = Cout; c.k = 3; c.stride = 1;
    e->make_mat(c.m, Cout, Cin * 9, 9, Cin, true);
    if (!c.m.w) { pd_set_error("allocation failed"); return 1; }
    PD_TRY(e->upload_rows(c.m, 0, w, Cout, true));
    if (bias) PD_TRY(e->upload_vec(c.m.bias, bias, Cout, false, 0));
    PD_TRY(e->fold_upconv(c.m));
    const int Ho = 2 * H, Wo = 2 * W;
    const int cpad = c.m.cin_pad, copad = round_up(Cout, 4);
    DevBuf in((size_t)B * H * W * cpad * dt_size(e->T)), out((size_t)B * Ho * Wo * copad * dt_size(e->T)),
        res((size_t)B * Ho * Wo * copad * dt_size(e->S));
    if (!in.p || !out.p || !res.p) { pd_set_error("allocation failed"); return 1; }
    PD_TRY(to_dev_nhwc(e, x, in.p, e->T, B, Cin, H, W, cpad));
    Act a, o, r;
    a.p = in.p; a.B = B; a.H = H; a.W = W; a.C = cpad; a.dt = e->T;
    o.p = out.p; o.B = B; o.H = Ho; o.W = Wo; o.C = copad; o.dt = e->T;
    r = o; r.p = res.p; r.dt = e->S;
    if (residual) PD_TRY(to_dev_nhwc(e, residual, res.p, e->S, B, Cout, Ho, Wo, copad));
    GemmCall call{.ups = 1, .R = residual ? &r : nullptr};
    PD_TRY(e->check_gemm(c.m, a, o, call));
    if (e->plan_gemm(e->fill_gemm(c.m, a, o, call), c.m, call).family != GEMM_UPFOLD) {
        pd_set_error("pd_op_conv2d_upfold: B %d Cin %d %dx%d Cout %d%s is not eligible for the four-phase upsample conv (mode, options, shape or epilogue)", B, Cin,
                     H, W, Cout, residual ? " + residual" : "");
        return 1;
    }
    PD_TRY(e->conv(c, a, o, call));
    return from_dev_nhwc(e, out.p, e->T, y, B, Cout, Ho, Wo, copad);
}

int pd_op_vae_downsample(pd_engine* e, const float* x, const float* w, const float* bias, int B, int C, int H, int W, float* y) {
    if (!e || !x || !w || !y) { pd_set_error("null argument"); return 1; }
    if (B < 1 || C < 1 || H < 2 || W < 2) { pd_set_error("pd_op_vae_downsample: need B, C >= 1 and H, W >= 2"); return 1; }
    HIP_OK(hipSetDevice(e->device));
    TempMat guard(e);
    ConvW c;
    c.cin = C; c.cout = C; c.k = 3; c.stride = 2; c.pad_shift = 1;
    e->make_mat(c.m, C, C * 9, 9, C, true);
    if (!c.m.w) { pd_set_error("allocation failed"); return 1; }
    PD_TRY(e->upload_rows(c.m, 0, w, C, true));
    if (bias) PD_TRY(e->upload_vec(c.m.bias, bias, C, false, 0));
    const int Ho = H / 2, Wo = W / 2;
    const int cpad = c.m.cin_pad, copad = round_up(C, 4);
    DevBuf in((size_t)B * H * W * cpad * dt_size(e->T)), out((size_t)B * Ho * Wo * copad * dt_size(e->T));
    if (!in.p || !out.p) { pd_set_error("allocation failed"); return 1; }
    PD_TRY(to_dev_nhwc(e, x, in.p, e->T, B, C, H, W, cpad));
    Act a, o;
    a.p = in.p; a.B = B; a.H = H; a.W = W; a.C = cpad; a.dt = e->T;
    o.p = out.p; o.B = B; o.H = Ho; o.W = Wo; o.C = copad; o.dt = e->T;
    PD_TRY(e->conv(c, a, o));
    return from_dev_nhwc(e, out.p, e->T, y, B, C, Ho, Wo, copad);
}

int pd_op_freeu_concat(pd_engine* e, const float* h, const float* h_add, const float* skip, const float* skip_add, int B, int C_h,
                       int C_skip, int H, int W, int skip_B, int skip_add_B, float s, float b, float* y) {
    if (!e || !h || !skip || !y) { pd_set_error("null argument"); return 1; }
    if (B < 1 || H < 1 || W < 1 || C_h < 4 || C_skip < 4 || C_h % 4 || C_skip % 4) {
        pd_set_error("pd_op_freeu_concat: need B, H, W >= 1 and C_h, C_skip positive multiples of 4");
        return 1;
    }
    if ((skip_B != B && 2 * skip_B != B) || (skip_add && skip_add_B != B && 2 * skip_add_B != B)) {
        pd_set_error("pd_op_freeu_concat: skip_B / skip_add_B must be B or B / 2");
        return 1;
    }
    HIP_OK(hipSetDevice(e->device));
    const int dt = e->S;
    const size_t px = (size_t)H * W, es = dt_size(dt);
    DevBuf dh((size_t)B * px * C_h * es), dha((size_t)B * px * C_h * es), ds((size_t)skip_B * px * C_skip * es),
        dsa((size_t)(skip_add ? skip_add_B : 1) * px * C_skip * es), dy((size_t)B * px * (C_h + C_skip) * es);
    if (!dh.p || !dha.p || !ds.p || !dsa.p || !dy.p) { pd_set_error("allocation failed"); return 1; }
    PD_TRY(to_dev_nhwc(e, h, dh.p, dt, B, C_h, H, W, C_h));
    if (h_add) PD_TRY(to_dev_nhwc(e, h_add, dha.p, dt, B, C_h, H, W, C_h));
    PD_TRY(to_dev_nhwc(e, skip, ds.p, dt, skip_B, C_skip, H, W, C_skip));
    if (skip_add) PD_TRY(to_dev_nhwc(e, skip_add, dsa.p, dt, skip_add_B, C_skip, H, W, C_skip));
    if (launch_freeu_concat(dh.p, h_add ? dha.p : nullptr, ds.p, skip_add ? dsa.p : nullptr, dy.p, dt, B, H, W, C_h, C_skip, s, b,
                            e->stream, (long long)skip_B * px, skip_add ? (long long)skip_add_B * px : 0)) {
        pd_set_error("pd_op_freeu_concat: launch failed");
        return 1;
    }
    return from_dev_nhwc(e, dy.p, dt, y, B, C_h + C_skip, H, W, C_h + C_skip);
}

int pd_op_linear(pd_engine* e, const float* x, const float* w, const float* bias, int M, int K, int N, int geglu, int a_silu,
                 float* y) {
    pd_gemm_ex_args a{};
    a.x = x; a.w = w; a.bias = bias; a.M = M; a.K = K; a.N = N; a.act = geglu ? ACT_GEGLU : ACT_NONE; a.a_silu = a_silu; a.y = y;
    return pd_op_linear_ex(e, &a);
}

namespace {
int ex_dt(const pd_engine* e, int code) { return code == 1 ? e->T : code == 2 ? e->S : DT_F32; }
int put_flat(pd_engine* e, const std::vector<float>& host, void* dst, int dt) {
    DevBuf tmp(host.size() * 4);
    if (!tmp.p) { pd_set_error("allocation failed"); return 1; }
    HIP_OK(hipMemcpy(tmp.p, host.data(), host.size() * 4, hipMemcpyHostToDevice));
    if (launch_cast_rows(reinterpret_cast<const float*>(tmp.p), dst, dt, 1, (int)host.size(), (int)host.size(), e->stream)) { pd_set_error("cast launch failed"); return 1; }
    HIP_OK(hipStreamSynchronize(e->stream));
    return 0;
}
int get_flat(pd_engine* e, const void* src, int dt, std::vector<float>& host) {
    DevBuf tmp(host.size() * 4);
    if (!tmp.p) { pd_set_error("allocation failed"); return 1; }
    if (launch_nhwc_to_nchw(src, dt, reinterpret_cast<float*>(tmp.p), 1, 1, 1, (int)host.size(), 1, 1.f, e->stream)) { pd_set_error("cast launch failed"); return 1; }
    HIP_OK(hipStreamSynchronize(e->stream));
    HIP_OK(hipMemcpy(host.data(), tmp.p, host.size() * 4, hipMemcpyDeviceToHost));
    return 0;
}
}

int pd_op_linear_ex(pd_engine* e, pd_gemm_ex_args* g) {
    if (!e || !g || !g->x || !g->w || !g->y) { pd_set_error("null argument"); return 1; }
    const int M = g->M, K = g->K, N = g->N, act = g->act;
    if (M < 1 || K < 1 || N < 1) { pd_set_error("pd_op_linear_ex: need M, K, N >= 1"); return 1; }
    if (K % 8) { pd_set_error("K must be a multiple of 8"); return 1; }
    if (act < 0 || act > ACT_GATED_TANH_GELU) { pd_set_error("pd_op_linear_ex: act %d out of range", act); return 1; }
    const bool packed = act == ACT_GEGLU || act == ACT_GATED_TANH_GELU;
    const int tokens = g->rows_per_sample > 0 ? g->rows_per_sample : M;
    if (M % tokens) { pd_set_error("pd_op_linear_ex: M %d is no multiple of rows_per_sample %d", M, tokens); return 1; }
    const int B = M / tokens;
    const float scale = g->scale == 0.f ? 1.f : g->scale;
    const bool remap = g->c_sample_rows || g->a_sample_rows;
    const bool side = g->residual || g->rowvec || g->gate || g->vt_begin || remap || g->ldc_extra || g->out_dt;
    if (N % 4 && side) { pd_set_error("pd_op_linear_ex: N %d must be a multiple of 4 with anything beyond bias / activation", N); return 1; }
    if ((unsigned)g->res_dt > 2u || (unsigned)g->out_dt > 2u) { pd_set_error("pd_op_linear_ex: dtype codes are 0 fp32, 1 compute type, 2 stream type"); return 1; }
    if (g->vt_begin) {
        if (g->vt_begin < 0 || g->vt_begin % 4 || g->vt_begin >= N) { pd_set_error("pd_op_linear_ex: vt_begin %d must be a multiple of 4 in (0, N)", g->vt_begin); return 1; }
        if (!g->vt || g->vt_extra < 0 || g->vt_extra % 8 || g->vt_tok_off < 0) { pd_set_error("pd_op_linear_ex: V^T needs an output array, vt_extra a multiple of 8, vt_tok_off >= 0"); return 1; }
    } else if (g->vt_extra || g->vt_tok_off) { pd_set_error("pd_op_linear_ex: vt_extra / vt_tok_off without vt_begin"); return 1; }
    if (g->ldc_extra < 0 || g->ldc_extra % 4) { pd_set_error("pd_op_linear_ex: ldc_extra %d must be a non-negative multiple of 4", g->ldc_extra); return 1; }
    if (g->c_sample_rows ? (g->c_row_off < 0 || g->c_row_off + tokens > g->c_sample_rows) : g->c_row_off != 0) { pd_set_error("pd_op_linear_ex: c_row_off + tokens must fit c_sample_rows"); return 1; }
    if (g->a_sample_rows ? (g->a_row_off < 0 || g->a_row_off + tokens > g->a_sample_rows) : g->a_row_off != 0) { pd_set_error("pd_op_linear_ex: a_row_off + tokens must fit a_sample_rows"); return 1; }
    const bool mm = g->gate || remap || act == ACT_TANH_GELU || act == ACT_ERF_GELU;
    if (packed && (g->residual || g->rowvec || g->gate || g->vt_begin || remap || scale != 1.f || g->a_silu || g->ln_gamma)) {
        pd_set_error("pd_op_linear_ex: a GEGLU / gated tanh-GELU layer takes a bias and nothing else");
        return 1;
    }
    if (act == ACT_RELU && mm) { pd_set_error("pd_op_linear_ex: the ReLU instantiations carry no gate / row remap"); return 1; }
    if (g->vt_tok_off && !mm) { pd_set_error("pd_op_linear_ex: vt_tok_off exists in the instantiations with the gate / row remaps only"); return 1; }
    if (g->ln_gamma && (!g->ln_beta || K > 2048 || g->a_silu)) { pd_set_error("pd_op_linear_ex: the LayerNorm fold needs gamma and beta, K <= 2048, no a_silu"); return 1; }
    HIP_OK(hipSetDevice(e->device));
    TempMat guard(e);
    WMat m;
    const int wrows = packed ? 2 * N : N;
    e->make_mat(m, wrows, K, 1, K, true, packed);
    if (!m.w) { pd_set_error("allocation failed"); return 1; }
    PD_TRY(e->upload_rows(m, 0, g->w, wrows, false));
    if (g->bias) PD_TRY(e->upload_vec(m.bias, g->bias, wrows, packed, N));
    const int adt = g->a_silu ? DT_F32 : g->ln_gamma ? e->S : e->T, odt = ex_dt(e, g->out_dt), rdt = ex_dt(e, g->res_dt);
    const int Np = round_up(N, 4), ldc = Np + g->ldc_extra, ncol = g->vt_begin ? g->vt_begin : Np;
    const int arows = g->a_sample_rows ? B * g->a_sample_rows : M, crows = g->c_sample_rows ? B * g->c_sample_rows : M;
    const int nvt = g->vt_begin ? N - g->vt_begin : 0, vt_ld = round_up(g->vt_tok_off + tokens, 8) + g->vt_extra;
    const float nan = std::nanf("");
    auto arow = [&](int i) { return g->a_sample_rows ? (i / tokens) * g->a_sample_rows + g->a_row_off + i % tokens : i; };
    auto crow = [&](int i) { return g->c_sample_rows ? (i / tokens) * g->c_sample_rows + g->c_row_off + i % tokens : i; };
    const size_t ob = dt_size(odt), nc = (size_t)crows * ldc, nv = (size_t)B * nvt * vt_ld;
    DevBuf in((size_t)arows * K * dt_size(adt)), out(nc * ob), vt(nv * ob), res((size_t)M * Np * dt_size(rdt)), rv((size_t)B * Np * 4), gt((size_t)B * Np * 4);
    if (!in.p || !out.p || !vt.p || !res.p || !rv.p || !gt.p) { pd_set_error("allocation failed"); return 1; }
    {
        std::vector<float> h((size_t)arows * K, g->a_sample_rows ? nan : 0.f);
        for (int i = 0; i < M; ++i) memcpy(&h[(size_t)arow(i) * K], g->x + (size_t)i * K, (size_t)K * 4);
        PD_TRY(put_flat(e, h, in.p, adt));
    }
    auto pad_cols = [&](const float* src, int rows, void* dst, int dt) -> int {
// ... 720 lines not shown
```

### prompt-diffusion_amd/csrc/options.cpp

```cpp
#include <cstdio>
#include <cstring>

#include "engine.h"

static const OptionRow* find_option(const char* key) {
    for (const OptionRow& r : kOptions)
        if (!strcmp(key, r.key)) return &r;
    return nullptr;
}

static void set_profiling(pd_engine* e, bool on) {
    (void)hipStreamSynchronize(e->stream);
    e->profiling = on;
    e->prof.clear();
    e->ev_used = 0;
    if (!e->profiling) return;
    const int n = 64;
    std::vector<hipEvent_t> ev(2 * n);
    for (auto& x : ev) x = e->next_event();
    for (int i = 0; i < n; ++i) {
        (void)hipEventRecord(ev[2 * i], e->stream);
        (void)hipEventRecord(ev[2 * i + 1], e->stream);
    }
    (void)hipStreamSynchronize(e->stream);
    double tot = 0.0;
    int cnt = 0;
    for (int i = n / 2; i < n; ++i) {
        float t = 0.f;
        if (ev[2 * i] && ev[2 * i + 1] && hipEventElapsedTime(&t, ev[2 * i], ev[2 * i + 1]) == hipSuccess) { tot += t; ++cnt; }
    }
    e->prof_overhead_ms = cnt ? (float)(tot / cnt) : 0.f;
    e->ev_used = 0;
}

extern "C" {

int pd_set_option(pd_engine* e, const char* key, int64_t value) {
    if (!e || !key) { pd_set_error("null argument"); return 1; }
    if (!strcmp(key, "verbose")) { e->opt.verbose = (int)value; return 0; }
    e->clear_graphs();
    const OptionRow* r = find_option(key);
    if (!r) { pd_set_error("unknown option '%s'", key); return 1; }
    if (r->accepts && !r->accepts(value)) { pd_set_error("%s", r->range_error); return 1; }
    if (r->kind == OPT_COMMAND) { set_profiling(e, value != 0); return 0; }
    e->opt.*r->member = r->kind == OPT_BOOL ? value != 0 : r->kind == OPT_TRI ? (value < 0 ? -1 : value != 0) : (int)value;
    if (r->effect == OPT_FX_LN) e->ln_dirty = true;
    if (r->effect == OPT_FX_SD3_FP8) e->sd3_fp8_dirty = true;
    return 0;
}

int pd_get_option(pd_engine* e, const char* key, int64_t* value) {
    if (!e || !key || !value) { pd_set_error("null argument"); return 1; }
    const OptionRow* r = find_option(key);
    if (!r) { pd_set_error("unknown option '%s'", key); return 1; }
    *value = r->kind == OPT_COMMAND ? (e->profiling ? 1 : 0) : (int64_t)(e->opt.*r->member);
    return 0;
}

int pd_option_info(int32_t index, const char** key, int64_t* default_value) {
    if (index < 0 || index >= (int32_t)(sizeof(kOptions) / sizeof(kOptions[0]))) return 1;
    if (key) *key = kOptions[index].key;
    if (default_value) *default_value = kOptions[index].def;
    return 0;
}

int64_t pd_get_stat(pd_engine* e, const char* key) {
    if (!e || !key) return -1;
    if (!strcmp(key, "ncu")) return (int64_t)e->ncu;
    if (!strcmp(key, "graph_captures")) return (int64_t)e->graph_captures;
    if (!strcmp(key, "graph_replays")) return (int64_t)e->graph_replays;
    if (!strcmp(key, "workspace_bytes")) return (int64_t)e->arena.cap;
    if (!strcmp(key, "side_workspace_bytes")) return (int64_t)e->arena2.cap;
    if (!strcmp(key, "weight_bytes")) return (int64_t)e->weight_bytes;
    if (!strcmp(key, "launches")) return (int64_t)e->launches;
    if (!strcmp(key, "image_allocs")) return (int64_t)e->image_allocs;
    if (!strcmp(key, "canny_sweeps")) return (int64_t)e->canny_sweeps;
    if (!strcmp(key, "gn_from_slabs")) return (int64_t)e->gn_from_slabs;
    if (!strcmp(key, "vae_tiles")) return (int64_t)e->vae_tiles_run;
    if (!strcmp(key, "vae_flash_launches")) return (int64_t)e->vae_flash_launches;
    if (!strcmp(key, "ups_fold_launches")) return (int64_t)e->ups_fold_launches;
    if (!strcmp(key, "ring_launches")) return (int64_t)e->ring_launches;
    if (!strcmp(key, "gn_kernel")) {
        static_assert(GN_KIND_TWO_PASS == PD_GN_TWO_PASS && GN_KIND_LDS_SLAB == PD_GN_LDS_SLAB && GN_KIND_REGISTER == PD_GN_REGISTER, "pdengine.h");
        return (int64_t)e->gn_kernel;
    }
    if (!strcmp(key, "attn_kernel")) {
        static_assert(ATTN_KIND_GENERIC == PD_ATTN_GENERIC && ATTN_KIND_PIPELINED == PD_ATTN_PIPELINED, "pdengine.h");
        return (int64_t)e->attn_kernel;
    }
    if (!strcmp(key, "gemm_family")) {
        static_assert(GEMM_GEMV == PD_GEMM_GEMV && GEMM_PATCH1 == PD_GEMM_PATCH1 && GEMM_PATCH2 == PD_GEMM_PATCH2 && GEMM_PATCH4 == PD_GEMM_PATCH4 &&
                      GEMM_RING == PD_GEMM_RING && GEMM_IGEMM == PD_GEMM_IGEMM && GEMM_UPFOLD == PD_GEMM_UPFOLD, "pdengine.h");
        return (int64_t)e->gemm_family;
    }
    if (!strcmp(key, "gemm_tile")) return (int64_t)e->gemm_tile;
    if (!strcmp(key, "gemm_ring_tile")) return (int64_t)e->gemm_ring_tile;
    if (!strcmp(key, "gemm_splitk")) return (int64_t)e->gemm_splitk;
    if (!strcmp(key, "steps")) return (int64_t)e->ses.S;
    if (!strcmp(key, "cfg_shared")) return (int64_t)((e->ses.share_u ? 1 : 0) | (e->ses.share_c ? 2 : 0) | (e->ses.cn_cond_only ? 4 : 0));
    if (!strcmp(key, "lora_base_bytes")) return (int64_t)e->lora_bytes(true);
    if (!strcmp(key, "lora_bytes")) return (int64_t)e->lora_bytes(false);
    if (!strcmp(key, "lora_targets")) return (int64_t)e->lora.size();
    if (!strcmp(key, "event_overhead_ns")) return (int64_t)(e->prof_overhead_ms * 1e6f);
    return -1;
}

int pd_profile_read(pd_engine* e, int32_t klass, double* total_ms, int64_t* n_launches, double* flops) {
    if (!e) { pd_set_error("null engine"); return 1; }
    HIP_OK(hipStreamSynchronize(e->stream));
    if (e->stream2) HIP_OK(hipStreamSynchronize(e->stream2));
    double ms = 0.0, fl = 0.0;
    int64_t n = 0;
    for (auto& r : e->prof) {
        if (klass >= 0 && r.klass != klass) continue;
        float t = 0.f;
        if (r.a && r.b && hipEventElapsedTime(&t, r.a, r.b) == hipSuccess) {
            t -= e->prof_overhead_ms;
            ms += t > 0.f ? t : 0.f;
            fl += r.flops;
            ++n;
        }
    }
    if (total_ms) *total_ms = ms;
    if (n_launches) *n_launches = n;
    if (flops) *flops = fl;
    return 0;
}

int pd_profile_dump(pd_engine* e, const char* path) {
    if (!e || !path) { pd_set_error("null argument"); return 1; }
    HIP_OK(hipStreamSynchronize(e->stream));
    if (e->stream2) HIP_OK(hipStreamSynchronize(e->stream2));
    FILE* f = fopen(path, "w");
    if (!f) { pd_set_error("cannot open %s", path); return 1; }
    fprintf(f, "klass,M,N,K,taps,ms,flops\n");
    for (auto& r : e->prof) {
        float t = 0.f;
        if (r.a && r.b && hipEventElapsedTime(&t, r.a, r.b) == hipSuccess) {
            t -= e->prof_overhead_ms;
            fprintf(f, "%d,%d,%d,%d,%d,%.6f,%.0f\n", r.klass, r.M, r.N, r.K, r.taps, t > 0.f ? t : 0.f, r.flops);
        }
    }
    fclose(f);
    return 0;
}

}
```

### prompt-diffusion_amd/csrc/pd_common.h

```cpp
#pragma once
#include <hip/hip_runtime.h>
#include <stdint.h>
#include <stddef.h>

enum PdDType : int { DT_F32 = 0, DT_BF16 = 1, DT_F16 = 2, DT_FP8 = 4 };
static inline size_t dt_size(int dt) { return dt == DT_F32 ? 4 : dt == DT_FP8 ? 1 : 2; }
constexpr int PREC_F16X2 = 3;
constexpr int PREC_FP8 = 4;
constexpr bool prec_f32_storage(int P) { return P == DT_F32 || P == PREC_F16X2; }

typedef __attribute__((ext_vector_type(4))) float f32x4;
typedef __attribute__((__vector_size__(4 * sizeof(unsigned int)))) unsigned int u32x4;
typedef __attribute__((ext_vector_type(8))) __bf16 bf16x8;
typedef __attribute__((ext_vector_type(8))) _Float16 f16x8;

#if defined(__HIPCC__)
__device__ __forceinline__ float bf2f(uint16_t v) { return __uint_as_float(((uint32_t)v) << 16); }
__device__ __forceinline__ uint16_t f2bf(float f) {
    __bf16 b = (__bf16)f;
    return __builtin_bit_cast(uint16_t, b);
}
typedef __attribute__((ext_vector_type(2))) float f32x2_t;
typedef __attribute__((ext_vector_type(2))) __bf16 bf16x2_t;
__device__ __forceinline__ uint32_t pack2bf(float lo, float hi) {
// ... 152 lines not shown
    const float* gate;
    int gate_stride;
    int c_sample_rows, c_row_off, vt_tok_off;
    int a_sample_rows, a_row_off;
    const float* a_scale;
    const float* w_scale;
    const float* c_scale;
    int pad_shift;
    int dil_m1;
};

struct AttnParams {
    const void* Q; const void* K; const void* VT; void* O;
    int ldq, ldk, ldo;
    int vt_ld;
    long long q_bs, k_bs, vt_bs, o_bs;
    int Nq, Nk, heads, dh;
    float scale;
    int B;
    int legacy;
    int causal;
};

int launch_gemm(const GemmParams& p, int prec, hipStream_t s, hipEvent_t mid = nullptr, int* parts = nullptr);
int gemm_stats_parts(const GemmParams& p, int prec);
int gemm_launched_tile(const GemmParams& p, int prec);
int ring_gemm_stats_parts(const GemmParams& p, int prec, int tile);
bool ring_gemm_eligible(const GemmParams& p, int prec);
int launch_ring_gemm(const GemmParams& p, int prec, int tile, int ncu, hipStream_t s, int* parts = nullptr);
int launch_quant_rows(const void* src, int src_dt, int src_ld, void* dst, int dst_ld, float* scale, int rows, int K, hipStream_t s);
int launch_gemv(const float* a, int lda, const void* W, int w_dt, int Kpad, const float* bias, float* y, int ldy, int B, int N, int K,
                int a_silu, hipStream_t s);
int gemm_tiles(int M, int N);
int launch_splitk_finalize(const GemmParams& p, hipStream_t s);
int conv_patch_tiles(const GemmParams& p, int prec);
int launch_conv_patch(const GemmParams& p, int prec, hipStream_t s);
int launch_conv_patch2(const GemmParams& p, int prec, hipStream_t s);
bool conv_patch4_eligible(const GemmParams& p, int prec);
int launch_conv_patch4(const GemmParams& p, int prec, hipStream_t s);
bool conv_upfold_eligible(const GemmParams& p, int prec);
int conv_upfold_tiles(const GemmParams& p);
int launch_conv_upfold(const GemmParams& p, const void* w_up, int prec, hipStream_t s);
int launch_upfold_weights(const void* w, void* w_up, int dt, int N, int cin_pad, int Kpad, hipStream_t s);
enum { ATTN_KIND_GENERIC = 1, ATTN_KIND_PIPELINED = 2 };
int launch_attention(const AttnParams& p, int prec, hipStream_t s, int* kind = nullptr);
struct VaeAttnParams {
    const void* Q; const void* K; const void* VT; void* O;
    int ldq, ldk, ldo, vt_ld;
    long long q_bs, k_bs, vt_bs, o_bs;
    int B, N, C;
    float scale;
};
bool vae_attention_eligible(int prec, int C);
int launch_vae_attention(const VaeAttnParams& p, int prec, hipStream_t s);
int launch_attention_bias(const AttnParams& p, const float* relbias, int prec, hipStream_t s, int* kind = nullptr);
bool st_tail_eligible(int prec, int C, int heads, int rows_per_sample, int Nk);
size_t st_tail_weight_bytes();
size_t st_tail_vec_floats();
size_t st_tail_kv_bytes(int B, int Nk);
int st_tail_windows(int Nk);
double st_tail_flops(long long M, int Nk);
size_t st_front_weight_bytes();
size_t st_front_vec_floats();
double st_front_flops(long long M);
int launch_st_front_pack(const void* wpi, const void* wqkv_ln, int ld, const float* bpi, const float* bqkv_ln, void* wdst, float* vdst, hipStream_t s);
int launch_st_front(const void* x, const float* coef, void* h, void* qk, void* vt, const void* wpk, const float* vec, long long M, int rows_per_sample,
                    int vt_ld, int prec, hipStream_t s);
int launch_st_tail_pack(const void* wo1, const void* wq_ln, const void* wo2, const void* w1_ln, const void* w2, const void* wp, int ld_c, int ld_w2,
                        void* dst, hipStream_t s);
int launch_st_tail_vec(const float* bo1, const float* bq_ln, const float* bo2, const float* b1_ln, const float* b2, const float* bp, float* dst,
                       hipStream_t s);
int launch_st_tail_kv_pack(const void* K, const void* VT, void* dst, int B, int Nk, int lpad, hipStream_t s);
int launch_st_tail(const void* att, const void* h, const void* x_in, void* out, const void* wpk, const float* vec, const void* kvp, long long M,
                   int rows_per_sample, int Nk, int s_dt, float scale, int prec, hipStream_t s, long long in_rows = 0);
int launch_gn_stats(const void* x, int x_dt, double* partial, int B, int HW, int C, int groups, int nchunk, hipStream_t s);
int launch_gn_apply(const void* x, int x_dt, void* y, int y_dt, const double* partial, const float* gamma,
                    const float* beta, int B, int HW, int C, int groups, int nchunk, float eps, int silu, hipStream_t s);
enum { GN_KIND_TWO_PASS = 1, GN_KIND_LDS_SLAB = 2, GN_KIND_REGISTER = 3 };
int gn_fused_bundle(int x_dt, int HW, int C, int groups, bool reg);
int launch_gn_fused(const void* x, int x_dt, void* y, int y_dt, const float* gamma, const float* beta, int B, int HW, int C, int groups,
                    float eps, int do_silu, bool reg, hipStream_t s, int* kind = nullptr);
int launch_gn_fused_slabs(const float* slabs, int nslab, const float* bias, const float* rowvec, int rowvec_stride, int x_dt, void* y, int y_dt,
                          const float* gamma, const float* beta, int B, int HW, int C, int groups, float eps, int do_silu, bool reg, hipStream_t s, int* kind = nullptr);
int launch_gn_coef(const double* partial, const float* gamma, const float* beta, float* coef, int B, int HW, int C, int groups,
                   int nchunk, float eps, hipStream_t s);
int launch_row_stats(const void* x, int x_dt, float* stats, int rows, int C, hipStream_t s);
int launch_ln_fold(const void* W, void* Wout, int dt, int N, int K, int Kpad, const float* gamma, const float* beta, const float* bias_in,
                   float* colsum, float* bias_out, hipStream_t s);
int launch_layernorm(const void* x, int x_dt, void* y, int y_dt, const float* gamma, const float* beta,
                     int rows, int C, float eps, hipStream_t s);
int launch_nchw_to_nhwc(const float* in, void* out, int out_dt, int B, int C, int H, int W, int Cpad, hipStream_t s,
                        float scale = 1.0f, float shift = 0.0f);
int launch_softmax_rows(const float* in, void* out, int out_dt, int rows, int n, hipStream_t s);
int launch_embed_tokens(const int* ids, const void* tok, int tok_ld, const void* pos, int pos_ld, int dt, void* out, int out_dt,
                        int B, int L, int C, int vocab, hipStream_t s);
int launch_nhwc_to_nchw(const void* in, int in_dt, float* out, int B, int C, int H, int W, int Cpad, float scale, hipStream_t s);
int launch_vae_tile_gather(const float* in, void* out, int out_dt, const int* origins, int ntile, int B, int C, int H, int W, int th, int tw,
                           int Cpad, float scale, float shift, hipStream_t s);
struct VaeBlendParams {
    const float* tiles; const long long* tile_off; const int* rows; const int* cols; const float* wtab;
    float* out;
    int B, C, Cpad, H, W, nrow, ncol, limit, nchw;
};
int launch_vae_tile_blend(const VaeBlendParams& p, hipStream_t s);
int launch_embed_rows(const int* ids, const void* tok, int tok_ld, int dt, float* out, long long rows, int C, int vocab, hipStream_t s);
int launch_rmsnorm_rows(const float* x, void* y, int y_dt, const float* w, long long rows, int C, float eps, int rows_per_sample, int y_sample_rows,
                        int y_row_off, int y_ld, hipStream_t s);
int launch_t5_relbias(const int* bucket, const void* table, int ld, int dt, float* relbias, int heads, int n, hipStream_t s);
int launch_joint_write(const float* src, float* dst, int B, int rows_per_sample, int C, int width, int dst_sample_rows, int dst_ld, int c_off,
                       hipStream_t s);
int launch_eos_gather(const int* ids, const float* x, float* out, int B, int L, int C, int eos_id, hipStream_t s);
int launch_cast_rows(const float* in, void* out, int out_dt, long long rows, int C, int Cpad, hipStream_t s);
int launch_concat_add(const void* a, const void* a_add, const void* b, const void* b_add, void* out, int dt,
                      long long rows, int Ca, int Cb, hipStream_t s, long long b_rows = 0, long long b_add_rows = 0);
int launch_add_inplace(void* a, const void* b, int dt, long long n, hipStream_t s);
int launch_freeu_concat(const void* h, const void* h_add, const void* skip, const void* skip_add, void* out, int dt, int B, int H,
                        int W, int Ch, int Cs, float s, float b, hipStream_t st, long long skip_rows = 0, long long skip_add_rows = 0);
struct UpdateState {
    const void* eps; int eps_dt, eps_C;
    float* x_state; float* pred_x0; float* eps_guided; float* x_in;
    int B, HW, C, Cpad, use_cfg;
};
struct BlendCoef { float sa, sb; int last; };
struct BlendArgs { const float* z0; const float* ieps; const float* mask; BlendCoef coef; };
struct DdimCoef { float sqrt_one_minus_at, sqrt_at, sqrt_a_prev, dir_coef, sigma, cfg_scale; };
int launch_cfg_ddim(const UpdateState& u, const DdimCoef& k, const float* noise, float temperature, int do_update, const BlendArgs* bl,
                    hipStream_t s, const uint32_t* rng_state = nullptr, uint32_t draw = 0);
struct UnipcCoef { double alpha, sigma, c_last, c_m[4], p_x, p_m[3]; int corr, n_hist; float cfg_scale; };
int launch_cfg_unipc(const UpdateState& u, const UnipcCoef& k, double* last, double* m_out, const double* const hist[3],
                     const BlendArgs* bl, hipStream_t s);
struct LmsCoef { double alpha, sigma, c_x, c_m[4], q_x, q_m[4]; int data_pred, base_keep, store_keep, push, n_hist; float cfg_scale; double c_z; };
int launch_cfg_lms(const UpdateState& u, const LmsCoef& k, double* keep, double* m_out, const double* const hist[3], const BlendArgs* bl,
                   hipStream_t s, const uint32_t* rng_state = nullptr, uint32_t draw = 0);
int launch_init_latents(const float* z0, const float* eps, float sa, float sb, int pure, float* x_state, float* x_in, float* out_nchw,
                        int B, int dup, int C, int Cpad, int HW, hipStream_t s, const uint32_t* rng_state = nullptr,
                        float* eps_out = nullptr);
int launch_randn(const uint32_t* rng_state, uint32_t stream, uint32_t draw, int B, long long per_sample, float* out, hipStream_t s);
int launch_fill_random(void* p, int dt, long long n, float scale, float shift, uint64_t seed, hipStream_t s);
int launch_lora_merge(int dt, void* W, const void* W0, int rows, int row_off, int geglu_half, int Kpad, const float* UT,
                      const float* D, const float* scale, int R, hipStream_t s);
int launch_lora_form_delta(float* out, int rows, int Kpad, const float* UT1, const float* D1, const float* scale, float s, int R1,
                           const float* UT2, const float* D2, int R2, hipStream_t st);
int launch_lora_kron_delta(float* out, int rows, int Kpad, int cin, int cin_pad, int taps, const float* w1, const float* w2, float s, int a,
                           int b, hipStream_t st);
int launch_lora_form_apply(int dt, void* W, const void* W0, float* sum, const float* delta, const float* mag, int rows, int row_off,
                           int geglu_half, int Kpad, int first, int last, hipStream_t st);
int launch_vae_posterior(const void* mom, int mom_dt, int Cpad, const float* noise, float* out, int B, int z, int HW, int what, float scale,
                         hipStream_t s, const uint32_t* rng_state = nullptr, float shift = 0.0f);
int launch_hed_upload(const float* in, void* out, int out_dt, int B, int H, int W, int Cpad, hipStream_t s);
int launch_hed_stage_tail(const void* x, int dt, const float* sw, const float* sb, float* score, void* pooled, int B, int H, int W, int C,
                          hipStream_t s);
int launch_hed_fuse(const float* const scores[5], const float* cw, const float* cb, float* out, int B, int H, int W, int what, hipStream_t s);
int launch_mlsd_upload(const uint8_t* in, void* out, int out_dt, int B, int H, int W, hipStream_t s);
int launch_mlsd_dwconv(const void* x, void* y, int dt, const float* w, const float* bias, int B, int H, int W, int C, int stride, int in_relu6,
                       hipStream_t s);
int launch_mlsd_upcat(const void* x, int ldx, void* y, int ldy, int dt, int B, int h, int w, int C, hipStream_t s);
int launch_mlsd_tpmap(const float* x, float* tp, int B, int h, int w, hipStream_t s);
constexpr int MLSD_TOPK = 200;
int launch_mlsd_decode(const float* tp, unsigned long long* cand, int* ncand, int* segs, int* count, int B, int h, int w, float thr_v,
                       float thr_d, hipStream_t s);
int launch_mlsd_draw(const int* segs, const int* count, int max_segs, uint8_t* map, int B, int H, int W, hipStream_t s);
int launch_image_hpass(const uint8_t* src, uint8_t* out, const int* bounds, const int* kk, int ksize, long long rows, int Ws, int W,
                       hipStream_t s);
int launch_image_vpass(const uint8_t* src, float* dst, const int* bounds, const int* kk, int ksize, int Bs, int Hs, int H, int W, int B,
                       int C, int c_off, int tile, float mul, float add, hipStream_t s);
int launch_image_store(const float* src, uint8_t* dst, int B, int C, int H, int W, float mul, float add, int trunc, hipStream_t s);
// ... 44 lines not shown
```

### prompt-diffusion_amd/engine.py

```python
from __future__ import annotations

import collections
import ctypes as C
import os
from typing import Dict, Iterable, List, Optional, Sequence, Tuple

import numpy as np

from .weights import (CLIP_VIT_H14, CLIP_VIT_L14_SAFETY, IMAGE_ENCODER_PREFIX, SAFETY_PREFIX, ClipVisionConfig, ModelConfig, SD15,
                      clip_vision_param_shapes, fold_mlsd_state_dict, hed_key, safety_param_shapes)

PD_PREC_BF16, PD_PREC_F32, PD_PREC_F16, PD_PREC_F16X2 = 0, 1, 2, 3
PRECISIONS = {"bf16": PD_PREC_BF16, "f32": PD_PREC_F32, "fp32": PD_PREC_F32, "f16": PD_PREC_F16, "fp16": PD_PREC_F16,
              "f16x2": PD_PREC_F16X2}
PD_MEM_HOST, PD_MEM_DEVICE = 0, 1
PD_DT_F32, PD_DT_F16, PD_DT_BF16 = 0, 1, 2
PD_GET_LATENTS, PD_GET_PRED_X0, PD_GET_EPS = 0, 1, 2
PD_VAE_MEAN, PD_VAE_SAMPLE, PD_VAE_MOMENTS = 0, 1, 2
VAE_ENCODE_MODES = {"mean": PD_VAE_MEAN, "sample": PD_VAE_SAMPLE, "moments": PD_VAE_MOMENTS}
PD_HED_EDGE, PD_HED_SIDES = 0, 1
HED_OUTPUTS = {"edge": PD_HED_EDGE, "sides": PD_HED_SIDES}
PD_MLSD_TPMAP, PD_MLSD_SEGMENTS, PD_MLSD_LINES = 0, 1, 2
MLSD_OUTPUTS = {"tpmap": PD_MLSD_TPMAP, "segments": PD_MLSD_SEGMENTS, "lines": PD_MLSD_LINES}
MLSD_TOPK = 200
# ... 194 lines not shown
    lib.pd_vae_get_tiling.argtypes = [C.c_void_p, C.c_int32] + [C.POINTER(C.c_int32)] * 3 + [C.POINTER(C.c_double), C.POINTER(C.c_int32)]
    lib.pd_vae_tile_plan.argtypes = [C.c_int32] * 3 + [C.c_double, C.c_int32, C.c_int32] + [C.POINTER(C.c_int32)] * 3 + [C.c_void_p, C.c_int32]
    lib.pd_op_vae_tile_blend.argtypes = [C.c_void_p] * 3 + [C.c_int] * 6 + [C.c_void_p]
    lib.pd_hed_configure.argtypes = [C.c_void_p]
    lib.pd_hed_weights_missing.argtypes = [C.c_void_p]
    lib.pd_hed_detect.argtypes = [C.c_void_p, C.c_void_p] + [C.c_int32] * 5 + [C.c_void_p]
    lib.pd_text_weights_missing.argtypes = [C.c_void_p]
    lib.pd_text_encode.argtypes = [C.c_void_p, C.c_void_p, C.c_int32, C.c_int32, C.c_void_p]
    lib.pd_text_encode_ex.argtypes = [C.c_void_p, C.c_void_p, C.c_int32, C.c_int32, C.c_int32, C.c_void_p]
    lib.pd_eps.argtypes = [C.c_void_p] + [C.c_void_p] * 6 + [C.c_int32] * 4 + [C.c_void_p, C.c_void_p]
    lib.pd_eps_ctx.argtypes = [C.c_void_p] + [C.c_void_p] * 3 + [C.c_int32] + [C.c_void_p] * 3 + [C.c_int32] * 4 + [C.c_void_p, C.c_void_p]
    lib.pd_control_shape.argtypes = [C.c_void_p, C.c_int, C.c_int32, C.c_int32] + [C.POINTER(C.c_int32)] * 3
    lib.pd_ddim_sample.argtypes = [C.c_void_p, C.POINTER(pd_sample_args), C.c_int32, C.c_void_p, C.c_void_p]
    lib.pd_sample_begin.argtypes = [C.c_void_p, C.POINTER(pd_sample_args)]
    lib.pd_sample_step.argtypes = [C.c_void_p, C.c_int32]
    lib.pd_sample_get.argtypes = [C.c_void_p, C.c_int32, C.c_int32, C.c_void_p]
    lib.pd_sample_set_latents.argtypes = [C.c_void_p, C.c_int32, C.c_void_p]
    lib.pd_sample_eps_at.argtypes = [C.c_void_p, C.c_int64, C.c_void_p]
    lib.pd_sample_set_guidance.argtypes = [C.c_void_p, C.c_float]
    lib.pd_sample_end.argtypes = [C.c_void_p]
    lib.pd_make_schedule.argtypes = [C.c_void_p, C.c_int32, C.c_float] + [C.c_void_p] * 5
    lib.pd_unipc_coefficients.argtypes = [C.POINTER(pd_config), C.POINTER(pd_unipc_args), C.c_void_p, C.c_int32, C.c_void_p]
    lib.pd_unipc_sample.argtypes = [C.c_void_p, C.POINTER(pd_sample_args), C.POINTER(pd_unipc_args), C.c_int32, C.c_void_p,
                                    C.c_void_p]
    lib.pd_sample_begin_unipc.argtypes = [C.c_void_p, C.POINTER(pd_sample_args), C.POINTER(pd_unipc_args)]
    lib.pd_lms_coefficients.argtypes = [C.POINTER(pd_config), C.POINTER(pd_lms_args), C.c_void_p, C.c_int32, C.c_void_p, C.c_void_p,
                                        C.POINTER(C.c_int32)]
    lib.pd_lms_sample.argtypes = [C.c_void_p, C.POINTER(pd_sample_args), C.POINTER(pd_lms_args), C.c_int32, C.c_void_p, C.c_void_p]
    lib.pd_sample_begin_lms.argtypes = [C.c_void_p, C.POINTER(pd_sample_args), C.POINTER(pd_lms_args)]
    lib.pd_sample_rows.argtypes = [C.c_void_p]
    lib.pd_sample_rows.restype = C.c_int32
    lib.pd_synchronize.argtypes = [C.c_void_p]
    lib.pd_stream.argtypes = [C.c_void_p]
    lib.pd_stream.restype = C.c_void_p
    lib.pd_wait_stream.argtypes = [C.c_void_p, C.c_void_p]
    lib.pd_set_option.argtypes = [C.c_void_p, C.c_char_p, C.c_int64]
    if hasattr(lib, "pd_get_option"):
        lib.pd_get_option.argtypes = [C.c_void_p, C.c_char_p, C.POINTER(C.c_int64)]
        lib.pd_option_info.argtypes = [C.c_int32, C.POINTER(C.c_char_p), C.POINTER(C.c_int64)]
    lib.pd_comm_new_id.argtypes = [C.c_void_p]
    lib.pd_comm_init.argtypes = [C.c_void_p, C.c_void_p, C.c_int32, C.c_int32]
    lib.pd_comm_world.argtypes = [C.c_void_p, C.POINTER(C.c_int32), C.POINTER(C.c_int32)]
    lib.pd_comm_all_gather.argtypes = [C.c_void_p, C.c_void_p, C.c_void_p, C.c_int64, C.c_int32]
    lib.pd_comm_destroy.argtypes = [C.c_void_p]
    lib.pd_get_stat.argtypes = [C.c_void_p, C.c_char_p]
    lib.pd_get_stat.restype = C.c_int64
    lib.pd_bench_conv3x3.argtypes = [C.c_void_p] + [C.c_int32] * 6 + [C.POINTER(C.c_float)]
    lib.pd_bench_linear.argtypes = [C.c_void_p] + [C.c_int32] * 5 + [C.POINTER(C.c_float)]
    lib.pd_profile_dump.argtypes = [C.c_void_p, C.c_char_p]
    lib.pd_profile_read.argtypes = [C.c_void_p, C.c_int32, C.POINTER(C.c_double), C.POINTER(C.c_int64), C.POINTER(C.c_double)]
    fp = C.c_void_p
    lib.pd_op_conv2d.argtypes = [C.c_void_p, fp, fp, fp, fp] + [C.c_int] * 9 + [C.c_float, C.c_int, fp]
    if hasattr(lib, "pd_op_conv2d_upfold"):
        lib.pd_op_conv2d_upfold.argtypes = [C.c_void_p, fp, fp, fp, fp] + [C.c_int] * 5 + [fp]
    lib.pd_op_linear.argtypes = [C.c_void_p, fp, fp, fp] + [C.c_int] * 5 + [fp]
    if hasattr(lib, "pd_op_linear_ex"):
        lib.pd_op_linear_ex.argtypes = [C.c_void_p, C.POINTER(pd_gemm_ex_args)]
        lib.pd_op_conv2d_ex.argtypes = [C.c_void_p, fp, fp, fp, fp, fp] + [C.c_int] * 9 + [C.c_float, C.c_int, fp]
    lib.pd_op_linear_fp8.argtypes = [C.c_void_p, fp, fp, fp] + [C.c_int] * 4 + [fp]
    lib.pd_op_groupnorm.argtypes = [C.c_void_p, fp, fp, fp] + [C.c_int] * 4 + [C.c_float, C.c_int, fp]
    lib.pd_op_layernorm.argtypes = [C.c_void_p, fp, fp, fp, C.c_int, C.c_int, fp]
    lib.pd_op_groupnorm_slabs.argtypes = [C.c_void_p, fp, C.c_int, fp, fp, fp, fp] + [C.c_int] * 4 + [C.c_float, C.c_int, fp]
    lib.pd_op_groupnorm_coef.argtypes = [C.c_void_p, fp, fp, fp] + [C.c_int] * 4 + [C.c_float, fp]
    lib.pd_op_ln_linear.argtypes = [C.c_void_p, C.c_int] + [fp] * 9 + [C.c_int] * 3 + [fp, fp, C.POINTER(C.c_int), fp]
    lib.pd_op_attention.argtypes = [C.c_void_p, fp, fp, fp] + [C.c_int] * 4 + [fp]
    lib.pd_op_attention_ex.argtypes = [C.c_void_p, fp, fp, fp] + [C.c_int] * 6 + [C.c_float, fp, C.c_int, C.c_int, C.c_float, fp, C.POINTER(C.c_int64)]
    lib.pd_op_vae_attention.argtypes = [C.c_void_p, fp, fp, fp] + [C.c_int] * 3 + [fp]
    lib.pd_bench_vae_attention.argtypes = [C.c_void_p] + [C.c_int32] * 5 + [C.POINTER(C.c_float), C.POINTER(C.c_int64)]
    lib.pd_op_spatial_transformer.argtypes = [C.c_void_p, C.c_char_p, fp, fp] + [C.c_int] * 3 + [fp]
    lib.pd_op_spatial_transformer_ctx.argtypes = [C.c_void_p, C.c_char_p, fp, fp] + [C.c_int] * 4 + [fp]
    lib.pd_op_time_embed.argtypes = [C.c_void_p, C.c_int, C.c_void_p, C.c_int, fp, fp]
    lib.pd_op_vae_downsample.argtypes = [C.c_void_p, fp, fp, fp] + [C.c_int] * 4 + [fp]
    lib.pd_op_hed_stage_tail.argtypes = [C.c_void_p, fp, fp, fp] + [C.c_int] * 4 + [fp, fp]
    lib.pd_op_hed_fuse.argtypes = [C.c_void_p, fp, fp, fp] + [C.c_int] * 4 + [fp]
    lib.pd_read_weights.argtypes = [C.c_void_p, C.c_char_p, C.c_void_p]
    lib.pd_lora_add.argtypes = [C.c_void_p, C.c_int32, C.c_char_p, C.c_void_p, C.c_int32, C.c_int32, C.c_void_p,
                                C.POINTER(C.c_int64), C.c_int32]
    lib.pd_lora_add_ex.argtypes = [C.c_void_p, C.c_int32, C.c_char_p, C.POINTER(LoraFactors)]
    lib.pd_lora_set_scales.argtypes = [C.c_void_p, C.c_void_p, C.c_int32]
    lib.pd_lora_remove.argtypes = [C.c_void_p, C.c_int32]
    lib.pd_set_freeu.argtypes = [C.c_void_p] + [C.c_float] * 4
    lib.pd_get_freeu.argtypes = [C.c_void_p, C.POINTER(C.c_float)]
    lib.pd_op_freeu_concat.argtypes = [C.c_void_p, fp, fp, fp, fp] + [C.c_int] * 7 + [C.c_float, C.c_float, fp]
    lib.pd_philox4x32_10.argtypes = [C.POINTER(C.c_uint32)] * 3
    lib.pd_philox4x32_10.restype = None
    lib.pd_set_rng.argtypes = [C.c_void_p, C.c_uint64, C.c_uint64]
    lib.pd_get_rng.argtypes = [C.c_void_p, C.POINTER(C.c_uint64), C.POINTER(C.c_uint64)]
    lib.pd_randn.argtypes = [C.c_void_p, C.c_int32, C.c_int32, C.c_int32, C.c_int64, C.c_int32, C.c_void_p]
    lib.pd_resample_coefficients.argtypes = [C.c_int32, C.c_int32, C.c_int32, C.POINTER(C.c_int32), C.c_void_p, C.c_void_p]
    lib.pd_image_load.argtypes = [C.c_void_p, C.POINTER(pd_image_load_args)]
    if hasattr(lib, "pd_clip_vision_configure"):
        lib.pd_resample_coefficients_ex.argtypes = [C.c_int32, C.c_int32, C.c_int32, C.POINTER(C.c_int32), C.c_void_p, C.c_void_p]
        lib.pd_clip_preprocess.argtypes = [C.c_void_p, C.POINTER(pd_clip_preprocess_args)]
        lib.pd_clip_preprocess_geometry.argtypes = [C.c_int32] * 3 + [C.POINTER(C.c_int32)] * 4
        lib.pd_clip_patch_width.argtypes = [C.c_int32]
        lib.pd_clip_vision_configure.argtypes = [C.c_void_p, C.POINTER(pd_clip_vision_config)]
        lib.pd_clip_vision_weights_missing.argtypes = [C.c_void_p, C.c_char_p]
        lib.pd_clip_vision_forward.argtypes = [C.c_void_p, C.POINTER(pd_clip_vision_args)]
        lib.pd_safety_configure.argtypes = [C.c_void_p]
        lib.pd_safety_weights_missing.argtypes = [C.c_void_p]
        lib.pd_safety_check.argtypes = [C.c_void_p, C.c_void_p, C.c_int32, C.c_int32, C.c_void_p, C.c_void_p]
        lib.pd_safety_blank.argtypes = [C.c_void_p, C.c_void_p, C.c_int32, C.c_int64, C.c_void_p, C.c_int32, C.c_float]
    lib.pd_image_store.argtypes = [C.c_void_p, C.c_void_p] + [C.c_int32] * 5 + [C.c_float, C.c_float, C.c_int32, C.c_void_p, C.c_int32]
    lib.pd_canny.argtypes = [C.c_void_p, C.POINTER(pd_canny_args)]
    lib.pd_op_canny_hysteresis.argtypes = [C.c_void_p, C.c_void_p, C.c_int, C.c_int, C.c_int, C.c_int, C.c_void_p]
    lib.pd_mlsd_configure.argtypes = [C.c_void_p]
    lib.pd_mlsd_weights_missing.argtypes = [C.c_void_p]
    lib.pd_mlsd_detect.argtypes = [C.c_void_p, C.c_void_p] + [C.c_int32] * 5 + [C.c_float, C.c_float, C.c_void_p]
    lib.pd_mlsd_detect_ex.argtypes = [C.c_void_p, C.POINTER(pd_mlsd_args)]
    lib.pd_op_dwconv3x3.argtypes = [C.c_void_p, fp, fp, fp] + [C.c_int] * 6 + [fp]
    lib.pd_op_upcat_bilinear.argtypes = [C.c_void_p, fp] + [C.c_int] * 6 + [fp]
    lib.pd_op_conv2d_dilated.argtypes = [C.c_void_p, fp, fp, fp] + [C.c_int] * 7 + [fp]
    lib.pd_op_mlsd_decode.argtypes = [C.c_void_p, fp, C.c_int, C.c_int, C.c_int, C.c_float, C.c_float, C.c_void_p, C.c_void_p]
    lib.pd_op_draw_lines.argtypes = [C.c_void_p, C.c_void_p, C.c_void_p] + [C.c_int] * 4 + [C.c_void_p]
    lib.pd_op_sd3_update.argtypes = [C.c_void_p] + [C.c_void_p] * 5 + [C.c_int] * 5 + [C.c_float] * 3 + [C.c_int] * 3 + [C.c_void_p] * 2
    if path is None:
        _lib = lib
    return lib


EXPORTS = [
    "pd_last_error", "pd_abi_version", "pd_engine_create", "pd_engine_destroy", "pd_param_count", "pd_param_info",
    "pd_load_weights", "pd_init_random_weights", "pd_weights_missing", "pd_vae_weights_missing", "pd_vae_decode",
    "pd_vae_encode", "pd_vae_encoder_weights_missing", "pd_vae_set_tiling", "pd_vae_set_slicing", "pd_vae_get_tiling", "pd_vae_tile_plan",
    "pd_op_vae_tile_blend", "pd_eps", "pd_eps_ctx", "pd_control_shape", "pd_ddim_sample",
    "pd_sample_begin", "pd_sample_step", "pd_sample_get", "pd_sample_set_latents", "pd_sample_set_guidance", "pd_sample_eps_at", "pd_sample_end",
    "pd_unipc_coefficients", "pd_unipc_sample", "pd_sample_begin_unipc",
    "pd_lms_coefficients", "pd_lms_sample", "pd_sample_begin_lms", "pd_sample_rows",
    "pd_make_schedule", "pd_synchronize", "pd_stream", "pd_wait_stream", "pd_set_option", "pd_get_option", "pd_option_info", "pd_get_stat", "pd_bench_conv3x3", "pd_bench_linear", "pd_text_encode", "pd_text_encode_ex", "pd_text_weights_missing",
    "pd_profile_read", "pd_profile_dump", "pd_comm_new_id", "pd_comm_init", "pd_comm_world", "pd_comm_all_gather", "pd_comm_destroy",
    "pd_sd3_configure", "pd_sd3_weights_missing", "pd_sd3_forward", "pd_sd3_control", "pd_sd3_sample", "pd_sd3_sample_ex", "pd_sd3_down_proj",
    "pd_op_sd3_update",
    "pd_op_conv2d", "pd_op_conv2d_ex", "pd_op_conv2d_upfold", "pd_op_linear", "pd_op_linear_ex", "pd_op_linear_fp8", "pd_op_groupnorm", "pd_op_layernorm", "pd_op_groupnorm_slabs", "pd_op_groupnorm_coef", "pd_op_ln_linear", "pd_op_attention", "pd_op_attention_ex", "pd_op_spatial_transformer", "pd_op_spatial_transformer_ctx", "pd_op_time_embed",
    "pd_op_timestep_embedding_i", "pd_op_timestep_embedding_f", "pd_op_vae_downsample", "pd_read_weights", "pd_lora_add", "pd_lora_add_ex", "pd_lora_set_scales", "pd_lora_remove",
    "pd_set_freeu", "pd_get_freeu", "pd_op_freeu_concat",
    "pd_philox4x32_10", "pd_set_rng", "pd_get_rng", "pd_randn",
    "pd_hed_configure", "pd_hed_weights_missing", "pd_hed_detect", "pd_op_hed_stage_tail", "pd_op_hed_fuse",
    "pd_mlsd_configure", "pd_mlsd_weights_missing", "pd_mlsd_detect", "pd_mlsd_detect_ex", "pd_op_dwconv3x3", "pd_op_upcat_bilinear", "pd_op_conv2d_dilated",
    "pd_op_mlsd_decode", "pd_op_draw_lines",
    "pd_resample_coefficients", "pd_image_load", "pd_image_store", "pd_canny", "pd_op_canny_hysteresis",
    "pd_sd3_text_configure", "pd_sd3_text_weights_missing", "pd_sd3_encode_prompt", "pd_sd3_text_encoder", "pd_t5_relative_buckets",
    "pd_resample_coefficients_ex", "pd_clip_preprocess", "pd_clip_preprocess_geometry", "pd_clip_patch_width", "pd_clip_vision_configure",
    "pd_clip_vision_weights_missing", "pd_clip_vision_forward", "pd_safety_configure", "pd_safety_weights_missing", "pd_safety_check", "pd_safety_blank",
    "pd_sd3_vae_configure", "pd_sd3_vae_weights_missing", "pd_sd3_vae_config_layout", "pd_sd3_vae_decode", "pd_sd3_vae_encode", "pd_op_vae_attention", "pd_bench_vae_attention",
]


def option_table() -> List[Tuple[str, int]]:
    lib = load_library()
    rows, k, d = [], C.c_char_p(), C.c_int64()
    while not lib.pd_option_info(len(rows), C.byref(k), C.byref(d)):
        rows.append((k.value.decode(), int(d.value)))
    return rows


def philox4x32_10(counter: Sequence[int], key: Sequence[int]) -> Tuple[int, int, int, int]:
    lib = load_library()
    c = (C.c_uint32 * 4)(*[int(v) & 0xFFFFFFFF for v in counter])
    k = (C.c_uint32 * 2)(*[int(v) & 0xFFFFFFFF for v in key])
    out = (C.c_uint32 * 4)()
    lib.pd_philox4x32_10(c, k, out)
    return tuple(int(v) for v in out)


def _filter_code(filter) -> int:
    return RESAMPLE_FILTERS[filter] if isinstance(filter, str) else int(filter)


PD_VAE_SD15, PD_VAE_SD3 = 0, 1
VAE_TILE_DEFAULTS = {PD_VAE_SD15: 64, PD_VAE_SD3: 128}


class pd_vae_tile(C.Structure):
    _fields_ = [(n, C.c_int32) for n in ("y0", "x0", "h", "w", "oy", "ox", "oh", "ow", "th", "tw", "ev", "eh", "cls")] + [("reserved", C.c_int32 * 3)]


VaeTile = collections.namedtuple("VaeTile", "y0 x0 h w oy ox oh ow th tw ev eh cls")
VaeTilePlan = collections.namedtuple("VaeTilePlan", "rows cols classes tiles")
VaeTilingState = collections.namedtuple("VaeTilingState", "tiling slicing tile_latent overlap_factor tile_batch")


def vae_tile_plan(h: int, w: int, tile_latent: int = 64, overlap_factor: float = 0.25, u: int = 8, encode: bool = False) -> VaeTilePlan:
    lib = load_library()
    r, c, k = C.c_int32(), C.c_int32(), C.c_int32()
    args = (int(h), int(w), int(tile_latent), float(overlap_factor), int(u), int(bool(encode)))
    if lib.pd_vae_tile_plan(*args, C.byref(r), C.byref(c), C.byref(k), None, 0):
        raise PdError(lib.pd_last_error().decode())
    n = r.value * c.value
    buf = (pd_vae_tile * max(n, 1))()
    if n and lib.pd_vae_tile_plan(*args, C.byref(r), C.byref(c), C.byref(k), C.addressof(buf), n):
        raise PdError(lib.pd_last_error().decode())
    return VaeTilePlan(r.value, c.value, k.value, [VaeTile(*(getattr(buf[i], f) for f in VaeTile._fields)) for i in range(n)])


def resample_ksize(in_size: int, out_size: int, filter="lanczos") -> int:
    lib = load_library()
    ks = C.c_int32()
    if lib.pd_resample_coefficients(int(in_size), int(out_size), _filter_code(filter), C.byref(ks), None, None):
        raise PdError(lib.pd_last_error().decode(errors="replace"))
    return int(ks.value)


def resample_coefficients(in_size: int, out_size: int, filter="lanczos") -> Tuple[np.ndarray, np.ndarray]:
    lib = load_library()
    ks = C.c_int32(resample_ksize(in_size, out_size, filter))
    bounds = np.zeros((int(out_size), 2), np.int32)
    kk = np.zeros((int(out_size), ks.value), np.int32)
    if lib.pd_resample_coefficients(int(in_size), int(out_size), _filter_code(filter), C.byref(ks), bounds.ctypes.data, kk.ctypes.data):
        raise PdError(lib.pd_last_error().decode(errors="replace"))
    return bounds, kk


def resample_coefficients_ex(in_size: int, out_size: int, filter="bicubic") -> Tuple[np.ndarray, np.ndarray]:
    lib = load_library()
    code = RESAMPLE_FILTERS_EX[filter] if isinstance(filter, str) else int(filter)
    ks = C.c_int32()
    if lib.pd_resample_coefficients_ex(int(in_size), int(out_size), code, C.byref(ks), None, None):
        raise PdError(lib.pd_last_error().decode(errors="replace"))
# ... 1329 lines not shown
        return score, pooled

    def op_hed_fuse(self, scores, cw, cb, what: str = "edge"):
        maps = [np.ascontiguousarray(s, np.float32) for s in scores]
        if len(maps) != 5:
            raise ValueError("five score maps expected")
        B, H, W = maps[0].shape[0], maps[0].shape[-2], maps[0].shape[-1]
        for i, m in enumerate(maps):
            if m.size != B * (H >> i) * (W >> i) or m.shape[-1] != W >> i:
                raise ValueError(f"score map {i} must be [{B}, {H >> i}, {W >> i}]")
        flat = np.ascontiguousarray(np.concatenate([m.reshape(-1) for m in maps]))
        cw = np.ascontiguousarray(np.asarray(cw, np.float32).reshape(-1))
        cb = np.ascontiguousarray(np.asarray(cb, np.float32).reshape(-1))
        if cw.size != 5 or cb.size != 1:
            raise ValueError("cw must hold 5 values and cb one")
        out = np.empty((B, 5 if what == "sides" else 1, H, W), np.float32)
        self._check(self.lib.pd_op_hed_fuse(self._h, flat.ctypes.data, cw.ctypes.data, cb.ctypes.data, B, H, W, HED_OUTPUTS[what],
                                            out.ctypes.data))
        return out

    def op_dwconv3x3(self, x, w, b, stride: int = 1, in_relu6: bool = False):
        x = np.ascontiguousarray(x, np.float32)
        w = np.ascontiguousarray(np.asarray(w, np.float32).reshape(-1))
        b = np.ascontiguousarray(np.asarray(b, np.float32).reshape(-1))
        B, Cc, H, W = x.shape
        if w.size != Cc * 9 or b.size != Cc:
            raise ValueError("w must be [C, 1, 3, 3] and b [C]")
        y = np.empty((B, Cc, H // stride, W // stride), np.float32)
        self._check(self.lib.pd_op_dwconv3x3(self._h, x.ctypes.data, w.ctypes.data, b.ctypes.data, B, Cc, H, W, int(stride), int(bool(in_relu6)),
                                             y.ctypes.data))
        return y

    def op_upcat_bilinear(self, x, y, c_off: int):
        x = np.ascontiguousarray(x, np.float32)
        y = np.array(y, np.float32, order="C")
        B, Cc, h, w = x.shape
        if y.shape != (B, y.shape[1], 2 * h, 2 * w):
            raise ValueError(f"y must be [{B}, Cy, {2 * h}, {2 * w}]")
        self._check(self.lib.pd_op_upcat_bilinear(self._h, x.ctypes.data, B, Cc, h, w, int(y.shape[1]), int(c_off), y.ctypes.data))
        return y

    def op_conv2d_dilated(self, x, w, b, dilation: int, relu: bool = False):
        x = np.ascontiguousarray(x, np.float32); w = np.ascontiguousarray(w, np.float32)
        bb = None if b is None else np.ascontiguousarray(b, np.float32)
        B, Cin, H, W = x.shape
        y = np.empty((B, w.shape[0], H, W), np.float32)
        self._check(self.lib.pd_op_conv2d_dilated(self._h, x.ctypes.data, w.ctypes.data, None if bb is None else bb.ctypes.data, B, Cin, H, W,
                                                  int(w.shape[0]), int(dilation), int(bool(relu)), y.ctypes.data))
        return y

    def op_mlsd_decode(self, tp, thr_v: float, thr_d: float):
        tp = np.ascontiguousarray(tp, np.float32)
        B, nine, h, w = tp.shape
        if nine != 9:
            raise ValueError("tp must be [B, 9, h, w]")
        segs = np.zeros((B, MLSD_TOPK, 4), np.int32)
        count = np.zeros(B, np.int32)
        self._check(self.lib.pd_op_mlsd_decode(self._h, tp.ctypes.data, B, h, w, float(thr_v), float(thr_d), segs.ctypes.data, count.ctypes.data))
        return [segs[b, :int(count[b])].copy() for b in range(B)]

    def op_draw_lines(self, segs, H: int, W: int):
        segs = [np.asarray(s, np.int32).reshape(-1, 4) for s in segs]
        B, n = len(segs), max(1, max(len(s) for s in segs))
        flat = np.zeros((B, n, 4), np.int32)
        for b, s in enumerate(segs):
            flat[b, :len(s)] = s
        count = np.array([len(s) for s in segs], np.int32)
        out = np.empty((B, H, W), np.uint8)
        self._check(self.lib.pd_op_draw_lines(self._h, flat.ctypes.data, count.ctypes.data, B, n, int(H), int(W), out.ctypes.data))
        return out

    def op_freeu_concat(self, h, skip, s: float, b: float, h_add=None, skip_add=None):
        f = lambda a: None if a is None else np.ascontiguousarray(a, np.float32)
        h, skip, h_add, skip_add = f(h), f(skip), f(h_add), f(skip_add)
        B, Ch, H, W = h.shape
        Cs = skip.shape[1]
        y = np.empty((B, Ch + Cs, H, W), np.float32)
        ptr = lambda a: None if a is None else a.ctypes.data
        self._check(self.lib.pd_op_freeu_concat(self._h, ptr(h), ptr(h_add), ptr(skip), ptr(skip_add), B, Ch, Cs, H, W,
                                                skip.shape[0], 0 if skip_add is None else skip_add.shape[0], float(s), float(b),
                                                y.ctypes.data))
        return y

    def op_sd3_update(self, shape, v=None, x=None, z0=None, mask=None, eps=None, use_cfg: bool = False, guidance: float = 1.0,
                      dsigma: float = 0.0, sigma: float = 0.0, pure: bool = False, seeded: bool = False, want_x_in: bool = False):
        B, Cc, H, W = (int(s) for s in shape)
        f = lambda a, shp: None if a is None else np.ascontiguousarray(a, np.float32).reshape(shp)
        v = f(v, ((2 if use_cfg else 1) * B, Cc, H, W))
        x, z0, eps, mask = f(x, (B, Cc, H, W)), f(z0, (B, Cc, H, W)), f(eps, (B, Cc, H, W)), f(mask, (B, 1, H, W))
        ptr = lambda a: None if a is None else a.ctypes.data
        out = np.empty((B, Cc, H, W), np.float32)
        x_in = np.empty((2 * B, Cc, H, W), np.float32) if want_x_in else None
        self._check(self.lib.pd_op_sd3_update(self._h, ptr(v), ptr(x), ptr(z0), ptr(mask), ptr(eps), B, Cc, H, W, int(bool(use_cfg)),
                                              float(guidance), float(dsigma), float(sigma), int(bool(pure)), int(bool(seeded)), PD_MEM_HOST,
                                              ptr(out), ptr(x_in)))
        return (out, x_in) if want_x_in else out

    def op_spatial_transformer(self, prefix: str, x, context):
        x = np.ascontiguousarray(x, np.float32); ctx = np.ascontiguousarray(context, np.float32)
        B, Cc, H, W = x.shape
        L = self._context_len(ctx, B, "context")
        y = np.empty_like(x)
        self._check(self.lib.pd_op_spatial_transformer_ctx(self._h, prefix.encode(), x.ctypes.data, ctx.ctypes.data, B, H, W, L, y.ctypes.data))
        return y
```

Before: 7.351 images/sec.

## Fuse decoder skip concat (with control residual add) into GroupNorm input

In the UNet decoder, the concatenation of the upsampled hidden state with the skip connection (plus ControlNet residual adds) is no longer launched as a separate kernel when FreeU is off. Instead, the GroupNorm kernels (fused, register, and two-pass stats) read from the two sources, add the residuals, write the concatenated tensor as a side output, and compute statistics in the same pass. This removes one kernel launch and one read pass over the concat output for each decoder resblock. The cost is heavier GroupNorm kernels with extra template variants and strided reads. A fallback materialises the concat when no kernel variant supports the shape or when the GN-fused conv path is taken.

Measured after the change: 7.412 images/sec (median of 6 runs). About the same (+0.8%).

```diff
diff --git a/include/pdengine_ops.h b/include/pdengine_ops.h
--- a/include/pdengine_ops.h
+++ b/include/pdengine_ops.h
@@ -44,6 +44,9 @@
 int pd_op_vae_downsample(pd_engine* e, const float* x, const float* w, const float* bias, int B, int C, int H, int W, float* y);
 int pd_op_freeu_concat(pd_engine* e, const float* h, const float* h_add, const float* skip, const float* skip_add, int B, int C_h,
                        int C_skip, int H, int W, int skip_B, int skip_add_B, float s, float b, float* y);
+int pd_op_concat_groupnorm(pd_engine* e, const float* h, const float* h_add, const float* skip, const float* skip_add, const float* gamma,
+                           const float* beta, int B, int C_h, int C_skip, int H, int W, int skip_B, int skip_add_B, float eps, int silu,
+                           float* cat, float* y);
 int pd_op_hed_stage_tail(pd_engine* e, const float* x, const float* w, const float* bias, int B, int C, int H, int W, float* score,
                          float* pooled);
 int pd_op_hed_fuse(pd_engine* e, const float* scores, const float* cw, const float* cb, int B, int H, int W, int what, float* out);
diff --git a/prompt-diffusion_amd/csrc/engine.cpp b/prompt-diffusion_amd/csrc/engine.cpp
--- a/prompt-diffusion_amd/csrc/engine.cpp
+++ b/prompt-diffusion_amd/csrc/engine.cpp
@@ -964,17 +964,30 @@
     return gemm(c.m, in, out, call);
 }
 
-int pd_engine::gn_stats(const Act& x, int& nchunk) {
+int pd_engine::gn_stats(const Act& x, int& nchunk, const GnCatSrc* cat) {
     const int HW = x.H * x.W;
     nchunk = HW / 8;
     if (nchunk < 1) nchunk = 1;
     if (nchunk > 64) nchunk = 64;
     while ((size_t)x.B * nchunk * 32 * 2 * sizeof(double) > gn_partial_cap && nchunk > 1) nchunk /= 2;
-    PD_LAUNCH(this, launch_gn_stats(x.p, x.dt, gn_partial, x.B, HW, x.C, 32, nchunk, stream), "groupnorm stats launch failed (C=%d)", x.C);
-    return 0;
-}
-
-int pd_engine::groupnorm(const Act& x, Act& y, const float* g, const float* b, float eps, bool silu, const SlabDefer* from_slabs) {
+    PD_LAUNCH(this, cat ? launch_gn_stats_cat(*cat, x.dt, gn_partial, x.B, HW, 32, nchunk, stream)
+                        : launch_gn_stats(x.p, x.dt, gn_partial, x.B, HW, x.C, 32, nchunk, stream), "groupnorm stats launch failed (C=%d)", x.C);
+    return 0;
+}
+
+int pd_engine::materialise_cat(const Act& x, const GnCatSrc& c) {
+    const long long hw = (long long)x.H * x.W;
+    PD_LAUNCH(this, launch_concat_add(c.a, c.a_add, c.b, c.b_add, c.cat_out, x.dt, x.rows(), c.Ca, c.Cb, stream, c.b_samples * hw, c.b_add ? c.b_add_samples * hw : 0),
+              "concat launch failed");
+    return 0;
+}
+
+int pd_engine::groupnorm(const Act& x, Act& y, const float* g, const float* b, float eps, bool silu, const SlabDefer* from_slabs, const GnCatSrc* cat) {
+    if (cat && !(x.dt == y.dt && gn_cat_kind(*cat, x.dt, x.B, x.H * x.W, 32, opt.gn_single, opt.gn_reg))) {
+        PD_TRY(materialise_cat(x, *cat));
+        cat = nullptr;
+    }
+    if (cat && !arena.dry) ++gn_from_cat;
     if (from_slabs && from_slabs->active) {
         if (!(opt.gn_single && gn_fused_bundle(x.dt, x.H * x.W, x.C, 32, opt.gn_reg))) { pd_set_error("internal: deferred split-K slabs without the single-kernel GroupNorm"); return 1; }
         if (arena.dry) return 0;
@@ -989,12 +1002,13 @@
         return 0;
     }
     if (opt.gn_single && gn_fused_bundle(x.dt, x.H * x.W, x.C, 32, opt.gn_reg)) {
-        PD_LAUNCH(this, launch_gn_fused(x.p, x.dt, y.p, y.dt, g, b, x.B, x.H * x.W, x.C, 32, eps, silu ? 1 : 0, opt.gn_reg, stream, &gn_kernel),
+        PD_LAUNCH(this, cat ? launch_gn_fused_cat(*cat, x.dt, y.p, g, b, x.B, x.H * x.W, 32, eps, silu ? 1 : 0, opt.gn_reg, stream, &gn_kernel)
+                            : launch_gn_fused(x.p, x.dt, y.p, y.dt, g, b, x.B, x.H * x.W, x.C, 32, eps, silu ? 1 : 0, opt.gn_reg, stream, &gn_kernel),
                   "groupnorm (single kernel) launch failed (C=%d)", x.C);
         return 0;
     }
     int nchunk = 1;
-    PD_TRY(gn_stats(x, nchunk));
+    PD_TRY(gn_stats(x, nchunk, cat));
     if (arena.dry) return 0;
     ++launches;
     gn_kernel = GN_KIND_TWO_PASS;
@@ -1006,18 +1020,19 @@
 }
 
 int pd_engine::conv_gn(const ConvW& c, const Act& x, Act& out, const float* g, const float* b, float eps, bool silu, GemmCall call,
-                       const SlabDefer* in_slabs) {
+                       const SlabDefer* in_slabs, const GnCatSrc* cat) {
     call.stride = c.stride; call.pad_shift = c.pad_shift; call.dilation = c.dilation;
     const bool fuse = opt.gn_fuse && x.C == c.m.cin_pad && patch_unsplit(patch_tiles(fill_gemm(c.m, x, out, call)));
     if (!fuse) {
         const size_t mk = arena.mark();
         Act a = new_act(x.B, x.H, x.W, x.C, T);
-        PD_TRY(groupnorm(x, a, g, b, eps, silu, in_slabs));
+        PD_TRY(groupnorm(x, a, g, b, eps, silu, in_slabs, cat));
         PD_TRY(gemm(c.m, a, out, call));
         if (!(call.defer && call.defer->active)) arena.release(mk);
         return 0;
     }
     if (in_slabs && in_slabs->active) { pd_set_error("internal: deferred split-K slabs in front of a GroupNorm-fused conv"); return 1; }
+    if (cat) PD_TRY(materialise_cat(x, *cat));
     int nchunk = 1;
     PD_TRY(gn_stats(x, nchunk));
     const size_t mk = arena.mark();
@@ -1068,13 +1083,13 @@
     return 0;
 }
 
-int pd_engine::resblock(const ResW& r, const Act& x, Act& out, const float* embrow, int emb_stride) {
+int pd_engine::resblock(const ResW& r, const Act& x, Act& out, const float* embrow, int emb_stride, const GnCatSrc* cat) {
     out = new_act(x.B, x.H, x.W, r.cout, S);
     const size_t mk = arena.mark();
     Act h = new_act(x.B, x.H, x.W, r.cout, T);
     SlabDefer d;
     d.allow = opt.slab_gn && !opt.gn_fuse && opt.gn_single && h.dt == T && gn_fused_bundle(T, x.H * x.W, r.cout, 32, opt.gn_reg) > 0;
-    PD_TRY(conv_gn(r.conv1, x, h, r.gn1_g, r.gn1_b, r.eps, true, {.rowvec = embrow, .rowvec_stride = emb_stride, .defer = &d}));
+    PD_TRY(conv_gn(r.conv1, x, h, r.gn1_g, r.gn1_b, r.eps, true, {.rowvec = embrow, .rowvec_stride = emb_stride, .defer = &d}, nullptr, cat));
     Act skip = x;
     if (r.has_skip) {
         skip = new_act(x.B, x.H, x.W, r.cout, S);
@@ -1312,14 +1327,16 @@
         const Act* b_add = only_mid ? nullptr : &ses.control[nctl - 1 - (int)i];
         const int stage = (int)i / (cfg.num_res_blocks + 1);
         const bool fu = stage < 2 && freeu_on();
-        PD_LAUNCH(this,
-                  fu ? launch_freeu_concat(h.p, a_add ? a_add->p : nullptr, skip.p, b_add ? b_add->p : nullptr, cat.p, S, h.B, h.H, h.W, h.C, skip.C,
-                                           freeu[stage], freeu[2 + stage], stream, skip.rows(), b_add ? b_add->rows() : 0)
-                     : launch_concat_add(h.p, a_add ? a_add->p : nullptr, skip.p, b_add ? b_add->p : nullptr, cat.p, S, h.rows(), h.C, skip.C, stream,
-                                         skip.rows(), b_add ? b_add->rows() : 0),
-                  fu ? "FreeU concat launch failed" : "concat launch failed");
+        const GnCatSrc cs{h.p, a_add ? a_add->p : nullptr, skip.p, b_add ? b_add->p : nullptr, cat.p, h.C, skip.C, skip.B, b_add ? b_add->B : skip.B};
+        const bool defer_cat = !freeu_on();
+        if (fu)
+            PD_LAUNCH(this, launch_freeu_concat(h.p, a_add ? a_add->p : nullptr, skip.p, b_add ? b_add->p : nullptr, cat.p, S, h.B, h.H, h.W, h.C, skip.C,
+                                                freeu[stage], freeu[2 + stage], stream, skip.rows(), b_add ? b_add->rows() : 0),
+                      "FreeU concat launch failed");
+        else if (!defer_cat)
+            PD_TRY(materialise_cat(cat, cs));
         Act o;
-        PD_TRY(resblock(b.res, cat, o, emb_ptr(ses.emb_u, b.res, emb_row), emb_stride ? b.res.cout : 0));
+        PD_TRY(resblock(b.res, cat, o, emb_ptr(ses.emb_u, b.res, emb_row), emb_stride ? b.res.cout : 0, defer_cat ? &cs : nullptr));
         if (b.attn) {
             Act o2;
             PD_TRY(transformer(b.st, o, o2, ses.kv_u[b.st.kv_slot]));
diff --git a/prompt-diffusion_amd/csrc/engine.h b/prompt-diffusion_amd/csrc/engine.h
--- a/prompt-diffusion_amd/csrc/engine.h
+++ b/prompt-diffusion_amd/csrc/engine.h
@@ -487,6 +487,7 @@
     Session ses;
     long long launches = 0;
     long long gn_from_slabs = 0;
+    long long gn_from_cat = 0;
     long long ring_launches = 0;
     int gn_kernel = 0;
     long long ups_fold_launches = 0;
@@ -688,13 +689,15 @@
     int fold_layernorms();
     bool ln_dirty = true;
     bool st_tail_on(const STW& s, int rows_per_sample, int L) const;
-    int gn_stats(const Act& x, int& nchunk);
+    int gn_stats(const Act& x, int& nchunk, const GnCatSrc* cat = nullptr);
     int conv(const ConvW& c, const Act& in, Act& out, GemmCall call = {});
     int conv_gn(const ConvW& c, const Act& x, Act& out, const float* g, const float* b, float eps, bool silu, GemmCall call = {},
-                const SlabDefer* in_slabs = nullptr);
-    int groupnorm(const Act& x, Act& y, const float* g, const float* b, float eps, bool silu, const SlabDefer* from_slabs = nullptr);
+                const SlabDefer* in_slabs = nullptr, const GnCatSrc* cat = nullptr);
+    int groupnorm(const Act& x, Act& y, const float* g, const float* b, float eps, bool silu, const SlabDefer* from_slabs = nullptr,
+                  const GnCatSrc* cat = nullptr);
+    int materialise_cat(const Act& x, const GnCatSrc& cat);
     int layernorm(const Act& x, Act& y, const float* g, const float* b, float eps = 1e-5f);
-    int resblock(const ResW& r, const Act& x, Act& out, const float* embrow, int emb_stride);
+    int resblock(const ResW& r, const Act& x, Act& out, const float* embrow, int emb_stride, const GnCatSrc* cat = nullptr);
     int transformer(const STW& s, const Act& x, Act& out, const KVSlot& kv, int out_B = 0);
     int repeat_act(const Act& src, int reps, Act& dst);
     static Act batch_view(const Act& a, int first, int count);
diff --git a/prompt-diffusion_amd/csrc/norm.hip b/prompt-diffusion_amd/csrc/norm.hip
--- a/prompt-diffusion_amd/csrc/norm.hip
+++ b/prompt-diffusion_amd/csrc/norm.hip
@@ -16,11 +16,62 @@
     dq += refine ? (double)pq + p * (2.0 * d + np) : (double)q;
 }
 
-template <int XD>
+struct GnCatLane { const char* p0; const char* p1; char* out; size_t stride, ostride; };
+__device__ __forceinline__ GnCatLane gn_cat_lane(const GnCatSrc& src, int smp, int HW, int c0) {
+    const bool in_a = c0 < src.Ca;
+    const int Cs = in_a ? src.Ca : src.Cb, cs = in_a ? c0 : c0 - src.Ca;
+    const int s0 = in_a || smp < src.b_samples ? smp : smp - src.b_samples;
+    const int s1 = in_a || smp < src.b_add_samples ? smp : smp - src.b_add_samples;
+    const void* add = in_a ? src.a_add : src.b_add;
+    GnCatLane l;
+    l.p0 = reinterpret_cast<const char*>(in_a ? src.a : src.b) + ((size_t)s0 * HW * Cs + cs) * 2;
+    l.p1 = add ? reinterpret_cast<const char*>(add) + ((size_t)s1 * HW * Cs + cs) * 2 : nullptr;
+    l.out = reinterpret_cast<char*>(src.cat_out) + ((size_t)smp * HW * (src.Ca + src.Cb) + c0) * 2;
+    l.stride = (size_t)Cs * 2;
+    l.ostride = (size_t)(src.Ca + src.Cb) * 2;
+    return l;
+}
+template <int NW> __device__ __forceinline__ void ld_words(const char* q, unsigned (&w)[NW]) {
+    if constexpr (NW == 4) {
+        const uint4 t = *reinterpret_cast<const uint4*>(q);
+        w[0] = t.x; w[1] = t.y; w[2] = t.z; w[3] = t.w;
+    } else if constexpr (NW == 2) {
+        const uint2 t = *reinterpret_cast<const uint2*>(q);
+        w[0] = t.x; w[1] = t.y;
+    } else {
+        w[0] = *reinterpret_cast<const unsigned*>(q);
+    }
+}
+template <int NW> __device__ __forceinline__ void st_words(char* q, const unsigned (&w)[NW]) {
+    if constexpr (NW == 4) *reinterpret_cast<uint4*>(q) = make_uint4(w[0], w[1], w[2], w[3]);
+    else if constexpr (NW == 2) *reinterpret_cast<uint2*>(q) = make_uint2(w[0], w[1]);
+    else *reinterpret_cast<unsigned*>(q) = w[0];
+}
+template <int XD, int NW> __device__ __forceinline__ void gn_cat_add(unsigned (&w)[NW], const unsigned (&add)[NW]) {
+#pragma unroll
+    for (int k = 0; k < NW; ++k) {
+        float lo, hi, alo, ahi;
+        unpack2<XD>(w[k], lo, hi);
+        unpack2<XD>(add[k], alo, ahi);
+        w[k] = pack2<XD>(lo + alo, hi + ahi);
+    }
+}
+template <int XD, int NW> __device__ __forceinline__ void gn_cat_load(const GnCatLane& l, int p, unsigned (&w)[NW]) {
+    ld_words<NW>(l.p0 + (size_t)p * l.stride, w);
+    if (l.p1) {
+        unsigned add[NW];
+        ld_words<NW>(l.p1 + (size_t)p * l.stride, add);
+        gn_cat_add<XD, NW>(w, add);
+    }
+    st_words<NW>(l.out + (size_t)p * l.ostride, w);
+}
+
+template <int XD, bool CAT = false>
 __global__ __launch_bounds__(GN_THREADS) void gn_stats_kernel(const void* __restrict__ x, double* __restrict__ partial,
-                                                               int HW, int C, int groups, int nchunk) {
+                                                               int HW, int C, int groups, int nchunk, GnCatSrc cat) {
     constexpr bool XF32 = XD == DT_F32;
     constexpr int VEC = XF32 ? 4 : 8;
+    static_assert(!(CAT && XF32), "the concat source is a 2-byte form");
     __shared__ double s_sum[64], s_sq[64];
     const int b = blockIdx.y, chunk = blockIdx.x;
     const int tid = threadIdx.x;
@@ -43,10 +94,16 @@
             for (int j = 0; j < VEC; ++j) { ds[j] = 0.0; dq[j] = 0.0; }
             [[maybe_unused]] float pv[VEC], pq[VEC];
             int cnt = 0;
+            [[maybe_unused]] GnCatLane lane;
+            if constexpr (CAT) lane = gn_cat_lane(cat, b, HW, v * VEC);
             for (int p = p0 + pr; p < p1; p += rows_par) {
                 const size_t idx = ((size_t)b * HW + p) * C + (size_t)v * VEC;
                 float f[VEC];
-                if constexpr (XF32) {
+                if constexpr (CAT) {
+                    unsigned w[4];
+                    gn_cat_load<XD, 4>(lane, p, w);
+                    unpack8<XD>(make_uint4(w[0], w[1], w[2], w[3]), f);
+                } else if constexpr (XF32) {
                     const f32x4 t = *reinterpret_cast<const f32x4*>(reinterpret_cast<const float*>(x) + idx);
 #pragma unroll
                     for (int j = 0; j < 4; ++j) f[j] = t[j];
@@ -195,10 +252,12 @@
 
 struct GnSlabSrc { const float* slabs; long long slab_stride; const float* bias; const float* row; int nslab, row_stride; };
 
-template <int XD, int YD, bool SLAB = false>
+template <int XD, int YD, bool SLAB = false, bool CAT = false>
 __global__ __launch_bounds__(GNF_THREADS) void gn_fused_kernel(const void* __restrict__ x, void* __restrict__ y,
                                                                 const float* __restrict__ gamma, const float* __restrict__ beta,
-                                                                int HW, int C, int groups, int BC, float eps, int do_silu, GnSlabSrc src) {
+                                                                int HW, int C, int groups, int BC, float eps, int do_silu, GnSlabSrc src,
+                                                                GnCatSrc cat) {
+    static_assert(!(CAT && (SLAB || XD == DT_F32)), "the concat source is a 2-byte form of its own");
     constexpr bool XF32 = XD == DT_F32, YF32 = YD == DT_F32;
     constexpr int VEC = XF32 ? 4 : 8;
     constexpr int EX = XF32 ? 4 : 2;
@@ -221,9 +280,15 @@
     for (int j = 0; j < VEC; ++j) { ds[j] = 0.0; dq[j] = 0.0; s[j] = 0.f; q[j] = 0.f; }
     [[maybe_unused]] float pv[VEC], pq[VEC];
     int cnt = 0;
+    [[maybe_unused]] GnCatLane lane;
+    if constexpr (CAT) lane = gn_cat_lane(cat, b, HW, c0);
     for (int p = pr; p < HW; p += rows_par) {
         uint4 raw;
-        if constexpr (SLAB) {
+        if constexpr (CAT) {
+            unsigned w[4];
+            gn_cat_load<XD, 4>(lane, p, w);
+            raw = make_uint4(w[0], w[1], w[2], w[3]);
+        } else if constexpr (SLAB) {
             const float* sp = src.slabs + ((size_t)b * HW + p) * C + c0;
             float acc[VEC];
 #pragma unroll
@@ -488,10 +553,11 @@
 }
 
 
-template <int XD, int VB, int NL, bool SLAB>
+template <int XD, int VB, int NL, bool SLAB, bool CAT = false>
 __global__ __launch_bounds__(NL == 16 ? 512 : 1024) void gn_reg_kernel(const void* __restrict__ x, void* __restrict__ y, const float* __restrict__ gamma,
                                                        const float* __restrict__ beta, int HW, int C, int groups, int nv, float eps,
-                                                       int do_silu, GnSlabSrc src) {
+                                                       int do_silu, GnSlabSrc src, GnCatSrc cat) {
+    static_assert(!(CAT && SLAB), "one input form at a time");
     constexpr int EV = VB / 2;
     constexpr int NW = VB / 4;
     __shared__ double red[16][2];
@@ -503,8 +569,24 @@
     const int c0 = g * cpg + v * EV;
     unsigned raw[NL][NW];
     const char* xb = reinterpret_cast<const char*>(x) + ((size_t)b * HW * C + c0) * 2;
-#pragma unroll
-    for (int i = 0; i < NL; ++i) {
+    if constexpr (CAT) {
+        const GnCatLane lane = gn_cat_lane(cat, b, HW, c0);
+        unsigned add[NL][NW];
+#pragma unroll
+        for (int i = 0; i < NL; ++i) ld_words<NW>(lane.p0 + (size_t)(pr + 64 * i) * lane.stride, raw[i]);
+        if (lane.p1) {
+#pragma unroll
+            for (int i = 0; i < NL; ++i) ld_words<NW>(lane.p1 + (size_t)(pr + 64 * i) * lane.stride, add[i]);
+        }
+#pragma unroll
+        for (int i = 0; i < NL; ++i) {
+            if (lane.p1) gn_cat_add<XD, NW>(raw[i], add[i]);
+            st_words<NW>(lane.out + (size_t)(pr + 64 * i) * lane.ostride, raw[i]);
+        }
+    }
+    constexpr int NLOAD = CAT ? 0 : NL;
+#pragma unroll
+    for (int i = 0; i < NLOAD; ++i) {
         const int p = pr + 64 * i;
         if constexpr (SLAB) {
             static_assert(!SLAB || EV >= 4, "slab input comes in 4-channel pieces");
@@ -610,19 +692,19 @@
     return 0;
 }
 
-template <bool SLAB>
+template <bool SLAB, bool CAT = false>
 static int launch_gn_reg(const void* x, int dt, void* y, const float* gamma, const float* beta, int B, int HW, int C, int groups, float eps,
-                         int do_silu, const GnSlabSrc& src, hipStream_t s) {
+                         int do_silu, const GnSlabSrc& src, hipStream_t s, const GnCatSrc& cat = GnCatSrc{}) {
     const int vb = gn_reg_vb(dt, dt, HW, C, groups, true);
     if (!vb) return 1;
     const int nv = (C / groups) * 2 / vb, nl = HW / 64;
     const dim3 grid(B * groups), block(64 * nv);
     bool done = false;
     auto go = [&](auto XD, auto VB, auto NL) {
-        if constexpr (SLAB && decltype(VB)::value < 8) return;
+        if constexpr ((SLAB || CAT) && decltype(VB)::value < 8) return;
         else {
-            hipLaunchKernelGGL((gn_reg_kernel<decltype(XD)::value, decltype(VB)::value, decltype(NL)::value, SLAB>), grid, block, 0, s, x, y, gamma, beta,
-                               HW, C, groups, nv, eps, do_silu, src);
+            hipLaunchKernelGGL((gn_reg_kernel<decltype(XD)::value, decltype(VB)::value, decltype(NL)::value, SLAB, CAT>), grid, block, 0, s, x, y, gamma, beta,
+                               HW, C, groups, nv, eps, do_silu, src, cat);
             done = true;
         }
     };
@@ -663,11 +745,11 @@
     if (groups > 64 || C % groups || C % 8) return 1;
     dim3 grid(nchunk, B);
     if (x_dt == DT_F32)
-        hipLaunchKernelGGL(gn_stats_kernel<DT_F32>, grid, dim3(GN_THREADS), 0, s, x, partial, HW, C, groups, nchunk);
+        hipLaunchKernelGGL(gn_stats_kernel<DT_F32>, grid, dim3(GN_THREADS), 0, s, x, partial, HW, C, groups, nchunk, GnCatSrc{});
     else if (x_dt == DT_F16)
-        hipLaunchKernelGGL(gn_stats_kernel<DT_F16>, grid, dim3(GN_THREADS), 0, s, x, partial, HW, C, groups, nchunk);
+        hipLaunchKernelGGL(gn_stats_kernel<DT_F16>, grid, dim3(GN_THREADS), 0, s, x, partial, HW, C, groups, nchunk, GnCatSrc{});
     else
-        hipLaunchKernelGGL(gn_stats_kernel<DT_BF16>, grid, dim3(GN_THREADS), 0, s, x, partial, HW, C, groups, nchunk);
+        hipLaunchKernelGGL(gn_stats_kernel<DT_BF16>, grid, dim3(GN_THREADS), 0, s, x, partial, HW, C, groups, nchunk, GnCatSrc{});
     return hipGetLastError() == hipSuccess ? 0 : 1;
 }
 
@@ -719,7 +801,7 @@
         static unsigned long long attr_done = 0;
         auto kfn = gn_fused_kernel<decltype(XD)::value, decltype(YD)::value>;
         if (ensure_dyn_smem(reinterpret_cast<const void*>(kfn), 104 * 1024, &attr_done)) { fail = true; return; }
-        hipLaunchKernelGGL(kfn, grid, dim3(GNF_THREADS), smem, s, x, y, gamma, beta, HW, C, groups, BC, eps, do_silu, GnSlabSrc{});
+        hipLaunchKernelGGL(kfn, grid, dim3(GNF_THREADS), smem, s, x, y, gamma, beta, HW, C, groups, BC, eps, do_silu, GnSlabSrc{}, GnCatSrc{});
     });
     return ok && !fail && hipGetLastError() == hipSuccess ? 0 : 1;
 }
@@ -745,9 +827,53 @@
         static unsigned long long attr_done = 0;
         auto kfn = gn_fused_kernel<decltype(XD)::value, decltype(YD)::value, true>;
         if (ensure_dyn_smem(reinterpret_cast<const void*>(kfn), 104 * 1024, &attr_done)) { fail = true; return; }
-        hipLaunchKernelGGL(kfn, grid, dim3(GNF_THREADS), smem, s, static_cast<const void*>(nullptr), y, gamma, beta, HW, C, groups, BC, eps, do_silu, src);
+        hipLaunchKernelGGL(kfn, grid, dim3(GNF_THREADS), smem, s, static_cast<const void*>(nullptr), y, gamma, beta, HW, C, groups, BC, eps, do_silu, src, GnCatSrc{});
     });
     return ok && !fail && hipGetLastError() == hipSuccess ? 0 : 1;
+}
+
+int gn_cat_kind(const GnCatSrc& src, int dt, int B, int HW, int groups, bool single, bool reg) {
+    const int C = src.Ca + src.Cb;
+    if ((dt != DT_F16 && dt != DT_BF16) || src.Ca <= 0 || src.Cb <= 0 || src.Ca % 8 || src.Cb % 8 || groups > 64 || C % groups) return 0;
+    if (!src.a || !src.b || !src.cat_out || src.b_samples < 1 || B > 2 * src.b_samples) return 0;
+    if (src.b_add && (src.b_add_samples < 1 || B > 2 * src.b_add_samples)) return 0;
+    if (single && reg && gn_reg_vb(dt, dt, HW, C, groups, true)) return GN_KIND_REGISTER;
+    if (single && gn_slab_bundle(dt, HW, C, groups)) return GN_KIND_LDS_SLAB;
+    return GN_KIND_TWO_PASS;
+}
+
+int launch_gn_fused_cat(const GnCatSrc& src, int dt, void* y, const float* gamma, const float* beta, int B, int HW, int groups, float eps,
+                        int do_silu, bool reg, hipStream_t s, int* kind) {
+    const int C = src.Ca + src.Cb;
+    const int k = gn_cat_kind(src, dt, B, HW, groups, true, reg);
+    if (kind) *kind = k == GN_KIND_TWO_PASS ? 0 : k;
+    if (k == GN_KIND_REGISTER) return launch_gn_reg<false, true>(nullptr, dt, y, gamma, beta, B, HW, C, groups, eps, do_silu, GnSlabSrc{}, s, src);
+    if (k != GN_KIND_LDS_SLAB) return 1;
+    const int BC = gn_slab_bundle(dt, HW, C, groups);
+    const size_t smem = (size_t)HW * BC * 2 + (GNF_THREADS / 64) * 4 * 2 * sizeof(double);
+    const dim3 grid(B * (C / BC));
+    bool fail = false;
+    auto go = [&](auto XD) {
+        static unsigned long long attr_done = 0;
+        auto kfn = gn_fused_kernel<decltype(XD)::value, decltype(XD)::value, false, true>;
+        if (ensure_dyn_smem(reinterpret_cast<const void*>(kfn), 104 * 1024, &attr_done)) { fail = true; return; }
+        hipLaunchKernelGGL(kfn, grid, dim3(GNF_THREADS), smem, s, static_cast<const void*>(nullptr), y, gamma, beta, HW, C, groups, BC, eps, do_silu,
+                           GnSlabSrc{}, src);
+    };
+    if (dt == DT_F16) go(std::integral_constant<int, DT_F16>{});
+    else go(std::integral_constant<int, DT_BF16>{});
+    return !fail && hipGetLastError() == hipSuccess ? 0 : 1;
+}
+
+int launch_gn_stats_cat(const GnCatSrc& src, int dt, double* partial, int B, int HW, int groups, int nchunk, hipStream_t s) {
+    const int C = src.Ca + src.Cb;
+    if (!gn_cat_kind(src, dt, B, HW, groups, false, false)) return 1;
+    dim3 grid(nchunk, B);
+    if (dt == DT_F16)
+        hipLaunchKernelGGL((gn_stats_kernel<DT_F16, true>), grid, dim3(GN_THREADS), 0, s, static_cast<const void*>(nullptr), partial, HW, C, groups, nchunk, src);
+    else
+        hipLaunchKernelGGL((gn_stats_kernel<DT_BF16, true>), grid, dim3(GN_THREADS), 0, s, static_cast<const void*>(nullptr), partial, HW, C, groups, nchunk, src);
+    return hipGetLastError() == hipSuccess ? 0 : 1;
 }
 
 int launch_gn_coef(const double* partial, const float* gamma, const float* beta, float* coef, int B, int HW, int C, int groups,
diff --git a/prompt-diffusion_amd/csrc/ops_abi.cpp b/prompt-diffusion_amd/csrc/ops_abi.cpp
--- a/prompt-diffusion_amd/csrc/ops_abi.cpp
+++ b/prompt-diffusion_amd/csrc/ops_abi.cpp
@@ -163,6 +163,46 @@
         return 1;
     }
     return from_dev_nhwc(e, dy.p, dt, y, B, C_h + C_skip, H, W, C_h + C_skip);
+}
+
+int pd_op_concat_groupnorm(pd_engine* e, const float* h, const float* h_add, const float* skip, const float* skip_add, const float* gamma,
+                           const float* beta, int B, int C_h, int C_skip, int H, int W, int skip_B, int skip_add_B, float eps, int silu,
+                           float* cat, float* y) {
+    if (!e || !h || !skip || !gamma || !beta || !cat || !y) { pd_set_error("null argument"); return 1; }
+    const int Cc = C_h + C_skip;
+    if (B < 1 || H < 1 || W < 1 || C_h < 4 || C_skip < 4 || C_h % 4 || C_skip % 4 || Cc % 32) {
+        pd_set_error("pd_op_concat_groupnorm: need B, H, W >= 1, C_h, C_skip positive multiples of 4 and C_h + C_skip a multiple of 32");
+        return 1;
+    }
+    if ((skip_B != B && 2 * skip_B != B) || (skip_add && skip_add_B != B && 2 * skip_add_B != B)) {
+        pd_set_error("pd_op_concat_groupnorm: skip_B / skip_add_B must be B or B / 2");
+        return 1;
+    }
+    HIP_OK(hipSetDevice(e->device));
+    const int dt = e->S;
+    const size_t px = (size_t)H * W, es = dt_size(dt);
+    DevBuf dh((size_t)B * px * C_h * es), dha((size_t)B * px * C_h * es), ds((size_t)skip_B * px * C_skip * es),
+        dsa((size_t)(skip_add ? skip_add_B : 1) * px * C_skip * es), dc((size_t)B * px * Cc * es), dy((size_t)B * px * Cc * dt_size(e->T)),
+        g((size_t)Cc * 4 + 16), b((size_t)Cc * 4 + 16);
+    if (!dh.p || !dha.p || !ds.p || !dsa.p || !dc.p || !dy.p || !g.p || !b.p) { pd_set_error("allocation failed"); return 1; }
+    const GnCatSrc src{dh.p, h_add ? dha.p : nullptr, ds.p, skip_add ? dsa.p : nullptr, dc.p, C_h, C_skip, skip_B, skip_add ? skip_add_B : skip_B};
+    if (e->S != e->T || !gn_cat_kind(src, dt, B, H * W, 32, e->opt.gn_single, e->opt.gn_reg)) {
+        pd_set_error("pd_op_concat_groupnorm: no GroupNorm kernel builds the concat of %d + %d channels in this mode (2-byte storage, both parts multiples of 8)",
+                     C_h, C_skip);
+        return 1;
+    }
+    HIP_OK(hipMemcpy(g.p, gamma, (size_t)Cc * 4, hipMemcpyHostToDevice));
+    HIP_OK(hipMemcpy(b.p, beta, (size_t)Cc * 4, hipMemcpyHostToDevice));
+    PD_TRY(to_dev_nhwc(e, h, dh.p, dt, B, C_h, H, W, C_h));
+    if (h_add) PD_TRY(to_dev_nhwc(e, h_add, dha.p, dt, B, C_h, H, W, C_h));
+    PD_TRY(to_dev_nhwc(e, skip, ds.p, dt, skip_B, C_skip, H, W, C_skip));
+    if (skip_add) PD_TRY(to_dev_nhwc(e, skip_add, dsa.p, dt, skip_add_B, C_skip, H, W, C_skip));
+    Act a, o;
+    a.p = dc.p; a.B = B; a.H = H; a.W = W; a.C = Cc; a.dt = dt;
+    o = a; o.p = dy.p; o.dt = e->T;
+    PD_TRY(e->groupnorm(a, o, reinterpret_cast<float*>(g.p), reinterpret_cast<float*>(b.p), eps, silu != 0, nullptr, &src));
+    PD_TRY(from_dev_nhwc(e, dc.p, dt, cat, B, Cc, H, W, Cc));
+    return from_dev_nhwc(e, dy.p, e->T, y, B, Cc, H, W, Cc);
 }
 
 int pd_op_linear(pd_engine* e, const float* x, const float* w, const float* bias, int M, int K, int N, int geglu, int a_silu,
diff --git a/prompt-diffusion_amd/csrc/options.cpp b/prompt-diffusion_amd/csrc/options.cpp
--- a/prompt-diffusion_amd/csrc/options.cpp
+++ b/prompt-diffusion_amd/csrc/options.cpp
@@ -76,6 +76,7 @@
     if (!strcmp(key, "image_allocs")) return (int64_t)e->image_allocs;
     if (!strcmp(key, "canny_sweeps")) return (int64_t)e->canny_sweeps;
     if (!strcmp(key, "gn_from_slabs")) return (int64_t)e->gn_from_slabs;
+    if (!strcmp(key, "gn_from_cat")) return (int64_t)e->gn_from_cat;
     if (!strcmp(key, "vae_tiles")) return (int64_t)e->vae_tiles_run;
     if (!strcmp(key, "vae_flash_launches")) return (int64_t)e->vae_flash_launches;
     if (!strcmp(key, "ups_fold_launches")) return (int64_t)e->ups_fold_launches;
diff --git a/prompt-diffusion_amd/csrc/pd_common.h b/prompt-diffusion_amd/csrc/pd_common.h
--- a/prompt-diffusion_amd/csrc/pd_common.h
+++ b/prompt-diffusion_amd/csrc/pd_common.h
@@ -258,6 +258,11 @@
                     float eps, int do_silu, bool reg, hipStream_t s, int* kind = nullptr);
 int launch_gn_fused_slabs(const float* slabs, int nslab, const float* bias, const float* rowvec, int rowvec_stride, int x_dt, void* y, int y_dt,
                           const float* gamma, const float* beta, int B, int HW, int C, int groups, float eps, int do_silu, bool reg, hipStream_t s, int* kind = nullptr);
+struct GnCatSrc { const void* a; const void* a_add; const void* b; const void* b_add; void* cat_out; int Ca, Cb, b_samples, b_add_samples; };
+int gn_cat_kind(const GnCatSrc& src, int dt, int B, int HW, int groups, bool single, bool reg);
+int launch_gn_fused_cat(const GnCatSrc& src, int dt, void* y, const float* gamma, const float* beta, int B, int HW, int groups, float eps,
+                        int do_silu, bool reg, hipStream_t s, int* kind = nullptr);
+int launch_gn_stats_cat(const GnCatSrc& src, int dt, double* partial, int B, int HW, int groups, int nchunk, hipStream_t s);
 int launch_gn_coef(const double* partial, const float* gamma, const float* beta, float* coef, int B, int HW, int C, int groups,
                    int nchunk, float eps, hipStream_t s);
 int launch_row_stats(const void* x, int x_dt, float* stats, int rows, int C, hipStream_t s);
diff --git a/prompt-diffusion_amd/engine.py b/prompt-diffusion_amd/engine.py
--- a/prompt-diffusion_amd/engine.py
+++ b/prompt-diffusion_amd/engine.py
@@ -300,6 +300,8 @@
     lib.pd_set_freeu.argtypes = [C.c_void_p] + [C.c_float] * 4
     lib.pd_get_freeu.argtypes = [C.c_void_p, C.POINTER(C.c_float)]
     lib.pd_op_freeu_concat.argtypes = [C.c_void_p, fp, fp, fp, fp] + [C.c_int] * 7 + [C.c_float, C.c_float, fp]
+    if hasattr(lib, "pd_op_concat_groupnorm"):
+        lib.pd_op_concat_groupnorm.argtypes = [C.c_void_p, fp, fp, fp, fp, fp, fp] + [C.c_int] * 7 + [C.c_float, C.c_int, fp, fp]
     lib.pd_philox4x32_10.argtypes = [C.POINTER(C.c_uint32)] * 3
     lib.pd_philox4x32_10.restype = None
     lib.pd_set_rng.argtypes = [C.c_void_p, C.c_uint64, C.c_uint64]
@@ -351,7 +353,7 @@
     "pd_op_sd3_update",
     "pd_op_conv2d", "pd_op_conv2d_ex", "pd_op_conv2d_upfold", "pd_op_linear", "pd_op_linear_ex", "pd_op_linear_fp8", "pd_op_groupnorm", "pd_op_layernorm", "pd_op_groupnorm_slabs", "pd_op_groupnorm_coef", "pd_op_ln_linear", "pd_op_attention", "pd_op_attention_ex", "pd_op_spatial_transformer", "pd_op_spatial_transformer_ctx", "pd_op_time_embed",
     "pd_op_timestep_embedding_i", "pd_op_timestep_embedding_f", "pd_op_vae_downsample", "pd_read_weights", "pd_lora_add", "pd_lora_add_ex", "pd_lora_set_scales", "pd_lora_remove",
-    "pd_set_freeu", "pd_get_freeu", "pd_op_freeu_concat",
+    "pd_set_freeu", "pd_get_freeu", "pd_op_freeu_concat", "pd_op_concat_groupnorm",
     "pd_philox4x32_10", "pd_set_rng", "pd_get_rng", "pd_randn",
     "pd_hed_configure", "pd_hed_weights_missing", "pd_hed_detect", "pd_op_hed_stage_tail", "pd_op_hed_fuse",
     "pd_mlsd_configure", "pd_mlsd_weights_missing", "pd_mlsd_detect", "pd_mlsd_detect_ex", "pd_op_dwconv3x3", "pd_op_upcat_bilinear", "pd_op_conv2d_dilated",
@@ -1847,6 +1849,19 @@
                                                 y.ctypes.data))
         return y
 
+    def op_concat_groupnorm(self, h, skip, gamma, beta, h_add=None, skip_add=None, eps: float = 1e-5, silu: bool = False):
+        f = lambda a: None if a is None else np.ascontiguousarray(a, np.float32)
+        h, skip, h_add, skip_add, g, bt = f(h), f(skip), f(h_add), f(skip_add), f(gamma), f(beta)
+        B, Ch, H, W = h.shape
+        Cs = skip.shape[1]
+        cat = np.empty((B, Ch + Cs, H, W), np.float32)
+        y = np.empty_like(cat)
+        ptr = lambda a: None if a is None else a.ctypes.data
+        self._check(self.lib.pd_op_concat_groupnorm(self._h, ptr(h), ptr(h_add), ptr(skip), ptr(skip_add), ptr(g), ptr(bt), B, Ch, Cs, H, W,
+                                                    skip.shape[0], 0 if skip_add is None else skip_add.shape[0], float(eps), int(silu),
+                                                    cat.ctypes.data, y.ctypes.data))
+        return cat, y
+
     def op_sd3_update(self, shape, v=None, x=None, z0=None, mask=None, eps=None, use_cfg: bool = False, guidance: float = 1.0,
                       dsigma: float = 0.0, sigma: float = 0.0, pure: bool = False, seeded: bool = False, want_x_in: bool = False):
         B, Cc, H, W = (int(s) for s in shape)
```
